# henriChevreux/distillation_trajectories

Hardware: AMD Instinct MI355X
Metric: trajectory-timesteps/sec (B×T U-Net fwd) at 16×16 T=50 (higher is better)
Workload: dtype f32 (fp32-accurate; convolutions: exact 3-plane bf16 operand split on bf16 MFMA with fp32 accumulate, or native fp32 MFMA, chosen per layer)

## Files before the change

distillation_trajectories_amd/csrc/dt_conv.hip:

```cpp
#include "dt_conv_epilogue.h"

namespace dt {

template <int BM, int BN>
__global__ __launch_bounds__(256, 4) void conv_gemm_kernel(const ConvParams p) {
  constexpr ConvForm F = *find_conv_form(KIND_FP32, BM, BN);
  constexpr int WN = F.wn();
  constexpr int MI = F.mi(), NI = F.ni();
  constexpr int A_PER = BM / 64, B_PER = BN / 64;
  constexpr int STAGE = (BM + BN) * 16;
  constexpr int LDS_FLOATS = 2 * STAGE > F.stage_floats() ? 2 * STAGE : F.stage_floats();
  static_assert(F.wm() == 2 && WN == 2 && MI * 64 == BM && NI * 64 == BN && LDS_FLOATS >= F.stage_floats(), "wave layout, epilogue stage");
  __shared__ __attribute__((aligned(16))) float lds[LDS_FLOATS];

  const int tid = threadIdx.x, lane = tid & 63, wave = tid >> 6;
  const int wm = wave / WN, wn = wave % WN;
  const int half = lane >> 5, l31 = lane & 31;
  const int m0 = blockIdx.x * BM, n0 = blockIdx.y * BN;
  const int HW = p.H * p.W;
  const int CC = p.cin_p >> 4;

  int a_off[A_PER], a_off2[A_PER], a_y[A_PER], a_x[A_PER];
  bool a_ok[A_PER];
  int a_lds[A_PER];
#pragma unroll
  for (int j = 0; j < A_PER; ++j) {
    const int q = tid + j * 256, row = q >> 2, pslot = q & 3;
    const int lslot = pslot ^ ((row >> 2) & 3);
    const int m = m0 + row;
    a_ok[j] = m < p.M;
    const int mm = a_ok[j] ? m : 0;
    const int b = mm / HW, rem = mm - b * HW;
    a_y[j] = rem / p.W;
    a_x[j] = rem - a_y[j] * p.W;
    a_off[j] = mm * p.cin_p + lslot * 4;
    a_off2[j] = mm * p.cin2_p + lslot * 4;
    a_lds[j] = q * 4;
  }
  const float *wbase = p.w + (size_t)n0 * 16 + tid * 4;

  f32x16 acc[MI][NI];
#pragma unroll
  for (int mi = 0; mi < MI; ++mi)
#pragma unroll
    for (int ni = 0; ni < NI; ++ni)
#pragma unroll
      for (int r = 0; r < 16; ++r) acc[mi][ni][r] = 0.f;

  int a_row[MI], b_row[NI];
#pragma unroll
  for (int mi = 0; mi < MI; ++mi) a_row[mi] = wm * (MI * 32) + mi * 32 + l31;
#pragma unroll
  for (int ni = 0; ni < NI; ++ni) b_row[ni] = wn * (NI * 32) + ni * 32 + l31;

  const int n_main = (p.tap_hi - p.tap_lo) * CC / p.splits;
  const int n_iter = n_main + (p.in2 ? (p.cin2_p >> 4) : 0);
  int tap = p.tap_lo + (blockIdx.z * n_main) / CC, cc = (blockIdx.z * n_main) % CC;
  for (int it = -1; it < n_iter; ++it) {
    const bool more = it + 1 < n_iter;
    f32x4 ra[A_PER], rb[B_PER];
    if (more && it + 1 >= n_main) {
      const int c2 = it + 1 - n_main;
#pragma unroll
      for (int j = 0; j < A_PER; ++j)
        ra[j] = a_ok[j] ? *reinterpret_cast<const f32x4 *>(p.in2 + a_off2[j] + c2 * 16) : f32x4{0.f, 0.f, 0.f, 0.f};
      const float *wt = p.w2 + (size_t)n0 * 16 + tid * 4 + (size_t)c2 * p.n_p * 16;
#pragma unroll
      for (int j = 0; j < B_PER; ++j) rb[j] = *reinterpret_cast<const f32x4 *>(wt + j * 1024);
    } else if (more) {
      int dy = 0, dx = 0;
      if (p.ksize == 3) { dy = tap / 3 - 1; dx = tap - (tap / 3) * 3 - 1; }
      const int shift = (dy * p.W + dx) * p.cin_p + cc * 16;
#pragma unroll
      for (int j = 0; j < A_PER; ++j) {
        const int yy = a_y[j] + dy, xx = a_x[j] + dx;
        const bool ok = a_ok[j] && yy >= 0 && yy < p.H && xx >= 0 && xx < p.W;
        ra[j] = ok ? *reinterpret_cast<const f32x4 *>(p.in + a_off[j] + shift) : f32x4{0.f, 0.f, 0.f, 0.f};
      }
      const float *wt = wbase + (size_t)(tap * p.ccw + cc) * p.n_p * 16;
#pragma unroll
      for (int j = 0; j < B_PER; ++j) rb[j] = *reinterpret_cast<const f32x4 *>(wt + j * 1024);
      if (++cc == CC) { cc = 0; ++tap; }
    }
    if (it >= 0) {
      if (it == n_main && p.in2) conv_midpoint<MI, NI>(p, acc, n0, wn, l31);
      const float *A = lds + (it & 1) * STAGE, *B = A + BM * 16;
#pragma unroll
      for (int s = 0; s < 2; ++s) {
        f32x4 fa[MI], fb[NI];
#pragma unroll
        for (int mi = 0; mi < MI; ++mi)
          fa[mi] = *reinterpret_cast<const f32x4 *>(A + a_row[mi] * 16 + (((2 * s + half) ^ ((a_row[mi] >> 2) & 3)) << 2));
#pragma unroll
        for (int ni = 0; ni < NI; ++ni)
          fb[ni] = *reinterpret_cast<const f32x4 *>(B + b_row[ni] * 16 + (((2 * s + half) ^ ((b_row[ni] >> 2) & 3)) << 2));
#pragma unroll
        for (int i = 0; i < 4; ++i)
#pragma unroll
          for (int mi = 0; mi < MI; ++mi)
#pragma unroll
            for (int ni = 0; ni < NI; ++ni) {
              acc[mi][ni] = __builtin_amdgcn_mfma_f32_32x32x2f32(fa[mi][i], fb[ni][i], acc[mi][ni], 0, 0, 0);
            }
      }
    }
    if (more) {
      float *A = lds + ((it + 1) & 1) * STAGE, *B = A + BM * 16;
#pragma unroll
      for (int j = 0; j < A_PER; ++j) *reinterpret_cast<f32x4 *>(A + a_lds[j]) = ra[j];
#pragma unroll
      for (int j = 0; j < B_PER; ++j) *reinterpret_cast<f32x4 *>(B + (tid + j * 256) * 4) = rb[j];
    }
    __syncthreads();
  }

  conv_epilogue<BM, BN, 1>(p, acc, lds, m0, n0, wm, wn, half, l31);
}

int launch_splitk_epilogue(const ConvParams &p, hipStream_t s);

#define DT_GEMM_ROW(cls, kind, bm, bn, kc, wk) {{kind, bm, bn, kc, wk, cls}, conv_gemm_kernel<bm, bn>},
static const ConvKernel kGemmKernels[] = {DT_CONV_FORMS_FP32(DT_GEMM_ROW)};

int launch_conv(const ConvParams &p, hipStream_t s) {
  if (!p.in || !p.w || !p.scale || !p.shift || !p.out) return DT_E_NULL;
  if (p.cin_p % 16 || p.cout_p % 16 || p.n_p % kNPad || p.M <= 0) return DT_E_SHAPE;
  if ((long long)p.M * p.cin_p >= (1ll << 31) || (long long)p.M * p.cout_p * (p.n_dup > 1 ? p.n_dup : 1) >= (1ll << 31)) return DT_E_SHAPE;
  if (const int st = conv_admissible(p)) return st;
  {
    const double flops = 2.0 * p.M * (double)p.cout_real * ((double)p.cin_real * p.ksize * p.ksize + (p.in2 ? p.cin2_real : 0));
    ProfileScope prof(find_conv_form(p.kind, p.bm, p.bn)->cls, flops, 4.0 * p.M * ((double)p.cin_real + p.cout_real), s);
    if (p.kind == KIND_FP32) {
      conv_kernel_of(kGemmKernels, p).fn<<<dim3((p.M + p.bm - 1) / p.bm, p.n_p / p.bn, p.splits), 256, 0, s>>>(p);
      DT_LAUNCH_CHECK();
    } else if (const int st = is_strip(p.kind) ? launch_conv_strip(p, s) : launch_conv_bf16x6(p, s)) return st;
  }
  return p.splits > 1 ? launch_splitk_epilogue(p, s) : DT_OK;
}


bool conv_choice_valid(const ConvChoice &c, int slot, int n_p) {
  if (!find_conv_form(c.kind, c.bm, c.bn) || n_p % c.bn) return false;
  if (c.splits < 1 || c.splits > 9 || c.splits == 5 || c.splits == 6 || c.splits == 7) return false;
  return !c.fuse || (slot == 2 && c.splits == 1);
}

static ConvChoice heuristic_choice(int M, int n_p, int taps) {
  ConvChoice c{};
  c.bn = n_p % 128 == 0 ? 128 : 64;
  const long long blocks128 = (long long)((M + 127) / 128) * (n_p / c.bn);
  c.bm = blocks128 >= 512 ? 128 : 64;
  const long long blocks = (long long)((M + c.bm - 1) / c.bm) * (n_p / c.bn);
  c.splits = 1;
  if (taps == 9 && M <= kSplitMaxRows && blocks < 384) c.splits = blocks * 3 >= 384 ? 3 : 9;
  c.fuse = c.splits == 1;
  return c;
}

ConvChoice resolve_conv_choice(const ConvLayer &L, const ConvChoice *req, int precision) {
  ConvChoice c = req ? *req : heuristic_choice(L.M, L.n_p, L.splittable ? L.taps : 1);
  const int cc = L.cin_p >> 4;
  if (!req) {
    c.kind = precision == DT_PREC_FP32 ? KIND_FP32 : KIND_BF16;
    if (c.kind == KIND_BF16 && L.taps == 9 && strip_reaches(L.W)) {
      c.kind = KIND_STRIP;
      c.splits = c.splits == 9 ? (cc % 8 == 0 ? 8 : (cc % 4 == 0 ? 4 : 1)) : (c.splits == 3 ? (cc % 4 == 0 ? 4 : (cc % 2 == 0 ? 2 : 1)) : 1);
    }
  }
  if (c.kind == 2) c.kind = KIND_BF16;
  if (is_strip(c.kind) && (L.taps != 9 || !strip_reaches(L.W))) c.kind = KIND_BF16;
  if (c.kind == KIND_STRIPK && !find_conv_form(c.kind, c.bm, c.bn)) c.kind = KIND_STRIP2;
  if (c.bm == 256 && !find_conv_form(c.kind, c.bm, c.bn)) c.bm = 128;
  if (!L.splittable) c.splits = 1;
  const ConvForm *f = find_conv_form(c.kind, c.bm, c.bn);
  if (is_strip(c.kind) ? !chunks_fit(cc, pack_chunks(L.cin_p), c.splits * (f ? f->kc : 1)) : (L.taps * cc) % c.splits != 0)
    c.splits = 1;
  c.fuse = L.foldable && c.fuse && c.splits == 1;
  return c;
}

int conv_admissible(const ConvParams &p) {
  const int cc = p.cin_p >> 4;
  const ConvForm *f = find_conv_form(p.kind, p.bm, p.bn);
  if (!f || p.n_p % p.bn) return DT_E_ARG;
  if (p.splits < 1 || (p.splits > 1 && !p.slab)) return DT_E_ARG;
  if (p.ccw < cc || (p.in2 && p.ccw2 < (p.cin2_p >> 4))) return DT_E_ARG;
  if (p.in2 && (p.splits != 1 || !p.w2 || !p.bias2 || p.cin2_p % 16)) return DT_E_ARG;
  if (!is_strip(p.kind)) return (p.tap_hi - p.tap_lo) * cc % p.splits ? DT_E_ARG : DT_OK;
  if (p.ksize != 3 || p.tap_lo != 0 || p.tap_hi != 9 || !chunks_fit(cc, p.ccw, p.splits * f->kc)) return DT_E_ARG;
  if (p.in2 && !chunks_fit(p.cin2_p >> 4, p.ccw2, f->kc)) return DT_E_ARG;
  return f->reaches(p.W) ? DT_OK : DT_E_SHAPE;
}

template <int S>
__device__ inline float4 splitk_finish(const ConvParams &p, unsigned m, int n, size_t slab_stride) {
  const size_t o = (size_t)m * p.cout_p + n;
  float4 a;
  if (S > 0) {
    float4 part[S > 0 ? S : 1];
#pragma unroll
    for (int z = 0; z < S; ++z) part[z] = *reinterpret_cast<const float4 *>(p.slab + z * slab_stride + o);
    a = part[0];
#pragma unroll
    for (int z = 1; z < S; ++z) { a.x += part[z].x; a.y += part[z].y; a.z += part[z].z; a.w += part[z].w; }
  } else {
    a = *reinterpret_cast<const float4 *>(p.slab + o);
    for (int z = 1; z < p.splits; ++z) {
      const float4 b = *reinterpret_cast<const float4 *>(p.slab + z * slab_stride + o);
      a.x += b.x; a.y += b.y; a.z += b.z; a.w += b.w;
    }
  }
  const float4 sc = *reinterpret_cast<const float4 *>(p.scale + n), sh = *reinterpret_cast<const float4 *>(p.shift + n);
  float4 v = make_float4(a.x * sc.x + sh.x, a.y * sc.y + sh.y, a.z * sc.z + sh.z, a.w * sc.w + sh.w);
  if (p.relu) { v.x = fmaxf(v.x, 0.f); v.y = fmaxf(v.y, 0.f); v.z = fmaxf(v.z, 0.f); v.w = fmaxf(v.w, 0.f); }
  if (p.tb) {
    const float4 t = *reinterpret_cast<const float4 *>(p.tb + (size_t)(m / (unsigned)p.m_per_tb) * p.tb_stride + n);
    v.x += t.x; v.y += t.y; v.z += t.z; v.w += t.w;
  }
  if (p.add) {
    const float4 t = *reinterpret_cast<const float4 *>(p.add + o);
    v.x += t.x; v.y += t.y; v.z += t.z; v.w += t.w;
  }
  *reinterpret_cast<float4 *>(p.out + o) = v;
  return v;
}

template <int S, bool POOL>
__global__ __launch_bounds__(256) void splitk_epilogue_kernel(const ConvParams p) {
  const unsigned c4 = (unsigned)p.cout_p >> 2;
  const size_t slab_stride = (size_t)p.M * p.cout_p;
  if (!POOL) {
    const unsigned total = (unsigned)p.M * c4;
    const bool pow2 = (c4 & (c4 - 1)) == 0;
    const int sh4 = 31 - __builtin_clz(c4);
    for (unsigned i = blockIdx.x * blockDim.x + threadIdx.x; i < total; i += gridDim.x * blockDim.x) {
      const unsigned m = pow2 ? i >> sh4 : i / c4;
      splitk_finish<S>(p, m, (int)(i - m * c4) * 4, slab_stride);
    }
  } else {
    const unsigned Wo = (unsigned)p.W >> 1, Ho = (unsigned)p.H >> 1, HW = (unsigned)(p.H * p.W);
    const unsigned total = ((unsigned)p.M >> 2) * c4;
    for (unsigned i = blockIdx.x * blockDim.x + threadIdx.x; i < total; i += gridDim.x * blockDim.x) {
      const unsigned wq = i / c4;
      const int n = (int)(i - wq * c4) * 4;
      const unsigned xo = wq % Wo, r = wq / Wo;
      const unsigned yo = r % Ho, b = r / Ho;
      const unsigned m00 = b * HW + 2 * yo * (unsigned)p.W + 2 * xo;
      const float4 a = splitk_finish<S>(p, m00, n, slab_stride), bq = splitk_finish<S>(p, m00 + 1, n, slab_stride);
      const float4 c = splitk_finish<S>(p, m00 + p.W, n, slab_stride), d = splitk_finish<S>(p, m00 + p.W + 1, n, slab_stride);
      float4 mx;
      mx.x = fmaxf(fmaxf(a.x, bq.x), fmaxf(c.x, d.x)); mx.y = fmaxf(fmaxf(a.y, bq.y), fmaxf(c.y, d.y));
      mx.z = fmaxf(fmaxf(a.z, bq.z), fmaxf(c.z, d.z)); mx.w = fmaxf(fmaxf(a.w, bq.w), fmaxf(c.w, d.w));
      *reinterpret_cast<float4 *>(p.pool_out + (size_t)wq * p.cout_p + n) = mx;
    }
  }
}

template <bool POOL>
static int launch_splitk_epilogue_t(const ConvParams &p, hipStream_t s) {
  const size_t total = (size_t)(POOL ? p.M / 4 : p.M) * (p.cout_p / 4);
  const int blocks = (int)((total + 255) / 256 < 4096 ? (total + 255) / 256 : 4096);
  ProfileScope prof(KC_SPLITK_EPILOGUE, 0.0, 4.0 * p.M * p.cout_p * (p.splits + 1.0 + (POOL ? 0.25 : 0.0)), s);
  switch (p.splits) {
    case 2: splitk_epilogue_kernel<2, POOL><<<blocks, 256, 0, s>>>(p); break;
    case 3: splitk_epilogue_kernel<3, POOL><<<blocks, 256, 0, s>>>(p); break;
    case 4: splitk_epilogue_kernel<4, POOL><<<blocks, 256, 0, s>>>(p); break;
    case 8: splitk_epilogue_kernel<8, POOL><<<blocks, 256, 0, s>>>(p); break;
    case 9: splitk_epilogue_kernel<9, POOL><<<blocks, 256, 0, s>>>(p); break;
    default: splitk_epilogue_kernel<0, POOL><<<blocks, 256, 0, s>>>(p); break;
  }
  DT_LAUNCH_CHECK();
  return DT_OK;
}

int launch_splitk_epilogue(const ConvParams &p, hipStream_t s) {
  return p.pool_out ? launch_splitk_epilogue_t<true>(p, s) : launch_splitk_epilogue_t<false>(p, s);
}

__global__ void pack_conv_kernel(const float *__restrict__ w, float *__restrict__ wp, int cout, int cin, int ksize,
                                 int cin_p, int n_p, int split_c, int split_cp, size_t total) {
  for (size_t idx = blockIdx.x * (size_t)blockDim.x + threadIdx.x; idx < total; idx += (size_t)gridDim.x * blockDim.x) {
    const int pos = idx & 15;
    const size_t rowi = idx >> 4;
    const int n = rowi % n_p;
    const int kc = rowi / n_p;
    const int pslot = pos >> 2, e = pos & 3;
    const int lslot = pslot ^ ((n >> 2) & 3);
    const int k = kc * 16 + lslot * 4 + e;
    const int tap = k / cin_p, cp = k - tap * cin_p;
    int c = -1;
    if (cp < split_cp) { if (cp < split_c) c = cp; }
    else { const int cc = split_c + (cp - split_cp); if (cc < cin) c = cc; }
    float v = 0.f;
    if (n < cout && c >= 0) v = w[((size_t)n * cin + c) * (ksize * ksize) + tap];
    wp[idx] = v;
  }
}

int launch_pack_conv(const float *w, float *wp, int cout, int cin, int ksize, int cin_p, int n_p, int split_c,
                     int split_cp, hipStream_t s) {
  const size_t total = (size_t)ksize * ksize * cin_p * n_p;
  const int blocks = (int)((total + 255) / 256 < 4096 ? (total + 255) / 256 : 4096);
  pack_conv_kernel<<<blocks, 256, 0, s>>>(w, wp, cout, cin, ksize, cin_p, n_p, split_c, split_cp, total);
  DT_LAUNCH_CHECK();
  return DT_OK;
}

__global__ void fold_bn_kernel(const float *cb, const float *g, const float *b, const float *mean, const float *var,
                               float *scale, float *shift, int cout, int n_p) {
  const int n = blockIdx.x * blockDim.x + threadIdx.x;
  if (n >= n_p) return;
  float sc = 0.f, sh = 0.f;
  if (n < cout) {
    if (g) {
      sc = g[n] / sqrtf(var[n] + 1e-5f);
      sh = (cb[n] - mean[n]) * sc + b[n];
    } else {
      sc = 1.f;
      sh = cb[n];
    }
  }
  scale[n] = sc;
  shift[n] = sh;
}

int launch_fold_bn(const float *cb, const float *g, const float *b, const float *mean, const float *var, float *scale,
                   float *shift, int cout, int n_p, hipStream_t s) {
  fold_bn_kernel<<<(n_p + 255) / 256, 256, 0, s>>>(cb, g, b, mean, var, scale, shift, cout, n_p);
  DT_LAUNCH_CHECK();
  return DT_OK;
}

__global__ void pack_res3_kernel(const float *w, const float *b, float *w3, int cout, int C, int n_p) {
  const int n = blockIdx.x * blockDim.x + threadIdx.x;
  if (n >= n_p) return;
  float4 v = make_float4(0.f, 0.f, 0.f, 0.f);
  if (n < cout) {
    v.x = w[n * C];
    if (C > 1) v.y = w[n * C + 1];
    if (C > 2) v.z = w[n * C + 2];
    v.w = b[n];
  }
  *reinterpret_cast<float4 *>(w3 + 4 * n) = v;
}

int launch_pack_res3(const float *w, const float *b, float *w3, int cout, int C, int n_p, hipStream_t s) {
  if (C > 3) return DT_E_SHAPE;
  pack_res3_kernel<<<(n_p + 255) / 256, 256, 0, s>>>(w, b, w3, cout, C, n_p);
  DT_LAUNCH_CHECK();
  return DT_OK;
}

}
```

distillation_trajectories_amd/csrc/dt_conv_epilogue.h:

```cpp
#pragma once
#include "dt_internal.h"

namespace dt {

typedef float f32x16 __attribute__((ext_vector_type(16)));
typedef float f32x4 __attribute__((ext_vector_type(4)));

typedef __bf16 bf16x8 __attribute__((ext_vector_type(8)));
typedef __bf16 bf16x2 __attribute__((ext_vector_type(2)));
typedef unsigned u32x4 __attribute__((ext_vector_type(4)));

__device__ inline float bf16_to_f32(__bf16 v) { return (float)v; }

__device__ inline void split8(const f32x4 lo, const f32x4 hi, bf16x8 &p1, bf16x8 &p2, bf16x8 &p3) {
#pragma unroll
  for (int i = 0; i < 8; ++i) {
    const float a = i < 4 ? lo[i] : hi[i - 4];
    const __bf16 a1 = (__bf16)a;
    const float r1 = a - (float)a1;
    const __bf16 a2 = (__bf16)r1;
    const float r2 = r1 - (float)a2;
    p1[i] = a1; p2[i] = a2; p3[i] = (__bf16)r2;
  }
}

__device__ inline void mfma_bf16x6(f32x16 &acc, const bf16x8 (&fa)[3], const bf16x8 (&fb)[3]) {
  f32x16 c = acc;
  c = __builtin_amdgcn_mfma_f32_32x32x16_bf16(fa[2], fb[0], c, 0, 0, 0);
  c = __builtin_amdgcn_mfma_f32_32x32x16_bf16(fa[1], fb[1], c, 0, 0, 0);
  c = __builtin_amdgcn_mfma_f32_32x32x16_bf16(fa[0], fb[2], c, 0, 0, 0);
  c = __builtin_amdgcn_mfma_f32_32x32x16_bf16(fa[1], fb[0], c, 0, 0, 0);
  c = __builtin_amdgcn_mfma_f32_32x32x16_bf16(fa[0], fb[1], c, 0, 0, 0);
  c = __builtin_amdgcn_mfma_f32_32x32x16_bf16(fa[0], fb[0], c, 0, 0, 0);
  acc = c;
}

template <int BM, int BN, int WK, int MI, int NI>
__device__ inline void conv_epilogue(const ConvParams &p, f32x16 (&acc)[MI][NI], float *stage, int m0, int n0, int wm, int wn,
                                     int half, int l31, int wk = 0) {
  constexpr ConvForm F = *find_conv_layout(BM, BN, WK);
  static_assert(MI == F.mi() && NI == F.ni(), "accumulator tiles of the form");
  constexpr int WM = F.wm(), P = F.pitch(), C4 = BN / 4, U = WM * C4 / 8;
  constexpr int COPY = F.copy_floats();
  const int tid = threadIdx.x;
  const int HW = p.H * p.W;
  const bool pow2 = (p.W & (p.W - 1)) == 0 && (HW & (HW - 1)) == 0;
  const int w_sh = 31 - __builtin_clz(p.W), hw_sh = 31 - __builtin_clz(HW);
  auto div_hw = [&](int m) { return pow2 ? m >> hw_sh : m / HW; };
  auto div_w = [&](int r) { return pow2 ? r >> w_sh : r / p.W; };
  const bool slab_mode = p.splits > 1;
  const size_t slab_stride = (size_t)p.M * p.cout_p;
  const int c4 = tid % C4, row0 = tid / C4;
  const int n = n0 + c4 * 4;
  const bool n_ok = n < p.cout_p;
  const int nn = n_ok ? n : 0;
  auto unit = [&](int k) __attribute__((always_inline)) {
    const float *src = stage + (row0 + k * (256 / C4)) * P + c4 * 4;
    f32x4 v = *reinterpret_cast<const f32x4 *>(src);
#pragma unroll
    for (int c = 1; c < WK; ++c) v += *reinterpret_cast<const f32x4 *>(src + c * COPY);
    return v;
  };
  auto unit_row = [&](int mi, int k) { const int row = row0 + k * (256 / C4); return m0 + (row >> 5) * (MI * 32) + mi * 32 + (row & 31); };
  auto to_stage = [&](int mi) __attribute__((always_inline)) {
    __syncthreads();
#pragma unroll
    for (int ni = 0; ni < NI; ++ni)
#pragma unroll
      for (int r = 0; r < 16; ++r) {
        const int L = 4 * half + (r & 3) + 8 * (r >> 2);
        stage[wk * COPY + (wm * 32 + L) * P + wn * (NI * 32) + ni * 32 + l31] = acc[mi][ni][r];
      }
    __syncthreads();
  };

  if (slab_mode) {
    float *slab = p.slab + (size_t)blockIdx.z * slab_stride;
#pragma unroll
    for (int mi = 0; mi < MI; ++mi) {
      to_stage(mi);
#pragma unroll
      for (int k = 0; k < U; ++k) {
        const int m = unit_row(mi, k);
        if (n_ok && m < p.M)
          *reinterpret_cast<f32x4 *>(slab + (size_t)m * p.cout_p + n) = unit(k);
      }
    }
    return;
  }

  auto pool_pass = [&](int mi, float *pool_out, const float *src, int n_src, int src_pitch, size_t out_pitch) __attribute__((always_inline)) {
    __syncthreads();
    const int Wo = p.W >> 1;
    for (int q0 = tid; q0 < n_src * WM * 8 * C4; q0 += 256) {
      const int pass = q0 / (WM * 8 * C4), q = q0 - pass * (WM * 8 * C4);
      const int pp = q / C4, qc = q % C4, j = pp & 7;
      const int yy = pow2 ? j >> (w_sh - 1) : j / Wo, xx = j - yy * Wo;
      const int L0 = 2 * yy * p.W + 2 * xx;
      const int m = m0 + (pp >> 3) * (MI * 32) + mi * 32 + L0;
      const int qn = n0 + qc * 4;
      if (m >= p.M || qn >= p.cout_p || (pass && m < p.dup_skip)) continue;
      const float *s0 = src + pass * src_pitch + ((pp >> 3) * 32 + L0) * P + qc * 4;
      const f32x4 a = *reinterpret_cast<const f32x4 *>(s0), b = *reinterpret_cast<const f32x4 *>(s0 + P);
      const f32x4 c = *reinterpret_cast<const f32x4 *>(s0 + p.W * P), d = *reinterpret_cast<const f32x4 *>(s0 + (p.W + 1) * P);
      f32x4 mx;
#pragma unroll
      for (int e = 0; e < 4; ++e) mx[e] = fmaxf(fmaxf(a[e], b[e]), fmaxf(c[e], d[e]));
      const int bimg = div_hw(m), rem = m - bimg * HW;
      const int y = div_w(rem), x = rem - y * p.W;
      *reinterpret_cast<f32x4 *>(pool_out + pass * out_pitch + (((size_t)bimg * (p.H >> 1) + (y >> 1)) * Wo + (x >> 1)) * p.cout_p + qn) = mx;
    }
  };
  f32x4 w3r[4];
#pragma unroll
  for (int e = 0; e < 4; ++e) w3r[e] = p.x3 ? *reinterpret_cast<const f32x4 *>(p.w3 + 4 * (nn + e)) : f32x4{0.f, 0.f, 0.f, 0.f};
  auto x3_skip = [&](int m, int) __attribute__((always_inline)) {
    f32x4 r;
    const int img = div_hw(m), pix = m - img * HW;
    const float *xr = p.x3 + (size_t)(img < p.x3_imgs ? img : img % p.x3_imgs) * p.x3_c * p.x3_hw + pix;
    const float x0 = xr[0], x1 = p.x3_c > 1 ? xr[p.x3_hw] : 0.f, x2 = p.x3_c > 2 ? xr[2 * p.x3_hw] : 0.f;
#pragma unroll
    for (int e = 0; e < 4; ++e) {
      const f32x4 w3 = w3r[e];
      float rs = w3[3];
      rs = fmaf(x0, w3[0], rs);
      if (p.x3_c > 1) rs = fmaf(x1, w3[1], rs);
      if (p.x3_c > 2) rs = fmaf(x2, w3[2], rs);
      r[e] = rs;
    }
    return r;
  };

#pragma unroll
  for (int mi = 0; mi < MI; ++mi) {
    f32x4 v[U];
    int mrow[U];
    bool ok[U];
    to_stage(mi);
#pragma unroll
    for (int k = 0; k < U; ++k) {
      mrow[k] = unit_row(mi, k);
      ok[k] = n_ok && mrow[k] < p.M;
    }
#pragma unroll
    for (int k = 0; k < U; ++k) v[k] = unit(k);
    if (p.n_dup) {
      const f32x4 sc = *reinterpret_cast<const f32x4 *>(p.scale + nn), sh = *reinterpret_cast<const f32x4 *>(p.shift + nn);
      f32x4 rs[U];
      int cls[U], mc[U];
#pragma unroll
      for (int k = 0; k < U; ++k) {
        mc[k] = ok[k] ? mrow[k] : m0;
        const int pix = mc[k] - div_hw(mc[k]) * HW, y = div_w(pix), x = pix - y * p.W;
        cls[k] = 3 * (y == 0 ? 0 : (y == p.H - 1 ? 2 : 1)) + (x == 0 ? 0 : (x == p.W - 1 ? 2 : 1));
      }
#pragma unroll
      for (int k = 0; k < U; ++k) rs[k] = p.x3 ? x3_skip(mc[k], nn) : f32x4{0.f, 0.f, 0.f, 0.f};
      if (p.n_dup == 2 && p.dup_stage2 && p.pool_out) {
        float *stage2 = stage + WK * COPY;
        f32x4 b0[U], b1[U];
#pragma unroll
        for (int k = 0; k < U; ++k) {
          const unsigned r0 = (unsigned)mc[k] / (unsigned)p.m_per_tb;
          const unsigned r1 = (unsigned)(p.dup_rows + (mc[k] >= p.dup_skip ? mc[k] - p.dup_skip : mc[k])) / (unsigned)p.m_per_tb;
          b0[k] = *reinterpret_cast<const f32x4 *>(p.tbc + (size_t)r0 * p.tb_stride + cls[k] * p.cout_p + nn);
          b1[k] = *reinterpret_cast<const f32x4 *>(p.tbc + (size_t)r1 * p.tb_stride + cls[k] * p.cout_p + nn);
        }
#pragma unroll
        for (int k = 0; k < U; ++k) {
          f32x4 o0 = (v[k] + b0[k]) * sc + sh, o1 = (v[k] + b1[k]) * sc + sh;
          if (p.relu) {
#pragma unroll
            for (int e = 0; e < 4; ++e) { o0[e] = fmaxf(o0[e], 0.f); o1[e] = fmaxf(o1[e], 0.f); }
          }
          o0 += rs[k]; o1 += rs[k];
          if (ok[k] && !p.skip_out) {
            *reinterpret_cast<f32x4 *>(p.out + (size_t)mrow[k] * p.cout_p + n) = o0;
            if (mrow[k] >= p.dup_skip) *reinterpret_cast<f32x4 *>(p.out + ((size_t)p.dup_rows + mrow[k] - p.dup_skip) * p.cout_p + n) = o1;
          }
          *reinterpret_cast<f32x4 *>(stage + (row0 + k * (256 / C4)) * P + c4 * 4) = o0;
          *reinterpret_cast<f32x4 *>(stage2 + (row0 + k * (256 / C4)) * P + c4 * 4) = o1;
        }
        pool_pass(mi, p.pool_out, stage, 2, WK * COPY, (size_t)((p.dup_rows - p.dup_skip) >> 2) * p.cout_p);
        continue;
      }
      for (int pass = 0; pass < p.n_dup; ++pass) {
        if (pass && m0 < p.dup_skip) break;
        f32x4 o[U];
        const int shift = pass ? pass * p.dup_rows - p.dup_skip : 0;
#pragma unroll
        for (int k = 0; k < U; ++k) {
          o[k] = f32x4{0.f, 0.f, 0.f, 0.f};
          if (ok[k]) {
            const size_t mg = (size_t)shift + mrow[k];
            const unsigned tr = (unsigned)(shift + mrow[k]) / (unsigned)p.m_per_tb;
            const f32x4 b = *reinterpret_cast<const f32x4 *>(p.tbc + (size_t)tr * p.tb_stride + cls[k] * p.cout_p + n);
            o[k] = (v[k] + b) * sc + sh;
            if (p.relu) {
#pragma unroll
              for (int e = 0; e < 4; ++e) o[k][e] = fmaxf(o[k][e], 0.f);
            }
            o[k] += rs[k];
            if (!p.skip_out) *reinterpret_cast<f32x4 *>(p.out + mg * p.cout_p + n) = o[k];
          }
        }
        if (p.pool_out) {
          if (pass) __syncthreads();
#pragma unroll
          for (int k = 0; k < U; ++k) *reinterpret_cast<f32x4 *>(stage + (row0 + k * (256 / C4)) * P + c4 * 4) = o[k];
          pool_pass(mi, p.pool_out + (size_t)(shift >> 2) * p.cout_p, stage, 1, 0, 0);
        }
      }
      continue;
    }
    if (p.in2) {
      const f32x4 b2 = *reinterpret_cast<const f32x4 *>(p.bias2 + nn);
#pragma unroll
      for (int k = 0; k < U; ++k) v[k] += b2;
    } else {
      const f32x4 sc = *reinterpret_cast<const f32x4 *>(p.scale + nn), sh = *reinterpret_cast<const f32x4 *>(p.shift + nn);
#pragma unroll
      for (int k = 0; k < U; ++k) {
        v[k] = v[k] * sc + sh;
        if (p.relu) {
#pragma unroll
          for (int e = 0; e < 4; ++e) v[k][e] = fmaxf(v[k][e], 0.f);
        }
      }
    }
    if (p.tb) {
      f32x4 t[U];
#pragma unroll
      for (int k = 0; k < U; ++k) {
        t[k] = f32x4{0.f, 0.f, 0.f, 0.f};
        if (ok[k]) t[k] = *reinterpret_cast<const f32x4 *>(p.tb + (size_t)(mrow[k] / p.m_per_tb) * p.tb_stride + n);
      }
#pragma unroll
      for (int k = 0; k < U; ++k) v[k] += t[k];
    }
    if (p.add) {
      f32x4 a[U];
#pragma unroll
      for (int k = 0; k < U; ++k) {
        a[k] = f32x4{0.f, 0.f, 0.f, 0.f};
        if (ok[k]) a[k] = *reinterpret_cast<const f32x4 *>(p.add + (size_t)mrow[k] * p.cout_p + n);
      }
#pragma unroll
      for (int k = 0; k < U; ++k) v[k] += a[k];
    }
    if (p.x3) {
#pragma unroll
      for (int k = 0; k < U; ++k)
        if (ok[k]) v[k] += x3_skip(mrow[k], nn);
    }
    if (p.head_out) {
      f32x4 hw[3];
#pragma unroll
      for (int c = 0; c < 3; ++c) {
        hw[c] = f32x4{0.f, 0.f, 0.f, 0.f};
        if (c < p.head_c && n_ok) {
#pragma unroll
          for (int e = 0; e < 4; ++e)
            if (n + e < p.head_cin) hw[c][e] = p.head_w[c * p.head_cin + n + e];
        }
      }
#pragma unroll
      for (int k = 0; k < U; ++k) {
        float part[3];
#pragma unroll
        for (int c = 0; c < 3; ++c) {
          part[c] = 0.f;
#pragma unroll
          for (int e = 0; e < 4; ++e) part[c] = fmaf(hw[c][e], v[k][e], part[c]);
#pragma unroll
          for (int off = C4 / 2; off > 0; off >>= 1) part[c] += __shfl_xor(part[c], off, 64);
        }
        if (c4 == 0 && mrow[k] < p.M) {
          f32x4 o = {part[0] + p.head_b[0], 0.f, 0.f, 0.f};
          if (p.head_c > 1) o[1] = part[1] + p.head_b[1];
          if (p.head_c > 2) o[2] = part[2] + p.head_b[2];
          *reinterpret_cast<f32x4 *>(p.head_out + (size_t)mrow[k] * 4) = o;
        }
      }
      continue;
    }
#pragma unroll
    for (int k = 0; k < U; ++k)
      if (ok[k]) *reinterpret_cast<f32x4 *>(p.out + (size_t)mrow[k] * p.cout_p + n) = v[k];
    if (p.pool_out) {
#pragma unroll
      for (int k = 0; k < U; ++k) *reinterpret_cast<f32x4 *>(stage + (row0 + k * (256 / C4)) * P + c4 * 4) = v[k];
      pool_pass(mi, p.pool_out, stage, 1, 0, 0);
    }
  }
}

template <int MI, int NI>
__device__ inline void conv_midpoint(const ConvParams &p, f32x16 (&acc)[MI][NI], int n0, int wn, int l31) {
#pragma unroll
  for (int ni = 0; ni < NI; ++ni) {
    const int n = n0 + wn * (NI * 32) + ni * 32 + l31;
    const float sc = p.scale[n], sh = p.shift[n];
#pragma unroll
    for (int mi = 0; mi < MI; ++mi)
#pragma unroll
      for (int r = 0; r < 16; ++r) {
        const float v = acc[mi][ni][r] * sc + sh;
        acc[mi][ni][r] = p.relu ? fmaxf(v, 0.f) : v;
      }
  }
}

}
```

distillation_trajectories_amd/csrc/dt_internal.h:

```cpp
#pragma once
#include <hip/hip_runtime.h>
#include <stddef.h>
#include <stdint.h>

#include "../../include/dt_hip.h"
#include "dt_conv_forms.h"

#define DT_HIP_TRY(expr)                         \
  do {                                           \
    hipError_t _e = (expr);                      \
    if (_e != hipSuccess) return (int)_e;        \
  } while (0)
#define DT_LAUNCH_CHECK()                        \
  do {                                           \
    hipError_t _e = hipGetLastError();           \
    if (_e != hipSuccess) return (int)_e;        \
  } while (0)

namespace dt {

enum KernelClass {
  KC_SPLITK_EPILOGUE = KC_CONV_COUNT, KC_FIRST_CONV, KC_POOL, KC_UPCAT, KC_HEAD, KC_HEAD_UP, KC_TIME_BIAS, KC_UPDATE, KC_METRICS,
  KC_WASSERSTEIN, KC_RESAMPLE, KC_FUSED, KC_PAIR_METRICS,
  KC_COUNT
};
struct ProfileScope {
  ProfileScope(int cls, double flops, double bytes, hipStream_t s);
  ~ProfileScope();
  int slot;
  hipStream_t stream;
  void *end_event;
};

__device__ inline void bilinear_src(int dst, int in, int out, int &i0, int &i1, float &l0, float &l1) {
#pragma clang fp contract(off)
  const float scale = out > 1 ? (float)(in - 1) / (float)(out - 1) : 0.f;
  const float src = scale * (float)dst;
  i0 = (int)src;
  i1 = i0 + (i0 < in - 1 ? 1 : 0);
  l1 = src - (float)i0;
  l0 = 1.f - l1;
}
__device__ inline float bilinear_blend(float v00, float v01, float v10, float v11, float wy0, float wy1, float wx0, float wx1) {
  const float top = fmaf(wx1, v01, wx0 * v00), bot = fmaf(wx1, v11, wx0 * v10);
  return fmaf(wy1, bot, wy0 * top);
}

constexpr int kChanPad = 16;
constexpr int kNPad = 64;
constexpr int kBlocks = 8;
constexpr int kChunkPad = 4;

inline int round_up(int v, int m) { return (v + m - 1) / m * m; }
inline bool chunks_fit(int cc, int ccw, int div) { return div >= 1 && round_up(cc, div) <= ccw; }
inline int pack_chunks(int cin_p) { return round_up(cin_p, 16 * kChunkPad) >> 4; }

struct ConvParams {
  const float *in;
  const float *w;
  const float *scale;
  const float *shift;
  const float *tb;
  const float *add;
  float *out;
  int M, H, W;
  int cin_p, cout_p, n_p;
  int cin_real, cout_real;
  int ksize;
  int tap_lo, tap_hi;
  int relu;
  int tb_stride;
  int m_per_tb;
  int splits;
  float *slab;
  int bm, bn;
  int kind;
  const float *x3;
  const float *w3;
  int x3_hw, x3_imgs, x3_c;
  const float *in2;
  const float *w2;
  const float *bias2;
  int cin2_p, cin2_real;
  float *pool_out;
  const float *in_b, *in2_b;
  int cc_a, b_stride;
  const float *head_w, *head_b;
  float *head_out;
  int head_c, head_cin;
  const float *tbc;
  int n_dup, dup_rows;
  int dup_skip;
  int skip_out;
  int dup_stage2;
  int ccw, ccw2;
};

int launch_conv(const ConvParams &p, hipStream_t s);
int launch_conv_bf16x6(const ConvParams &p, hipStream_t s);
int launch_conv_strip(const ConvParams &p, hipStream_t s);
struct ConvKernel { ConvForm form; void (*fn)(ConvParams); };
template <size_t N>
inline const ConvKernel &conv_kernel_of(const ConvKernel (&table)[N], const ConvParams &p) {
  for (const ConvKernel &k : table)
    if (k.form.kind == p.kind && k.form.bm == p.bm && k.form.bn == p.bn) return k;
  return table[0];
}
int launch_pack_conv_bf16x3(const float *w_oihw, void *wp, int cout, int cin, int ksize, int cin_p, int cin_w, int n_p,
                            int split_c, int split_cp, hipStream_t s);
constexpr int kSplitMaxRows = 32768;

struct ConvChoice { int bm, bn, splits, kind, fuse; };
struct ConvLayer {
  int M, W;
  int n_p, cin_p;
  int taps;
  bool splittable;
  bool foldable;
};
inline bool strip_reaches(int W) { return find_conv_form(KIND_STRIP, 64, 64)->reaches(W); }
bool conv_choice_valid(const ConvChoice &c, int slot, int n_p);
ConvChoice resolve_conv_choice(const ConvLayer &L, const ConvChoice *req, int precision);
int conv_admissible(const ConvParams &p);

int launch_pack_conv(const float *w_oihw, float *wp, int cout, int cin, int ksize, int cin_p, int n_p,
                     int split_c, int split_cp, hipStream_t s);
int launch_fold_bn(const float *conv_b, const float *g, const float *b, const float *mean, const float *var,
                   float *scale, float *shift, int cout, int n_p, hipStream_t s);
int launch_pack_linear_rows(const float *w, const float *b, float *wp, float *bp, int out, int in, int out_p,
                            hipStream_t s);

int launch_first_conv(const float *x, const float *wf, const float *scale, const float *shift, const float *tb, int tb_stride,
                      int tb_div, float *out, int B, int n_pass, int C, int H, int W, int cout, int cout_p, hipStream_t s);
int launch_pack_first_conv(const float *w_oihw, float *wf, int cout, int C, int cout_p, hipStream_t s);
int launch_pack_tap_major(const float *w_oihw, float *w2t, int cout, int cin, int cp, hipStream_t s);
int launch_maxpool(const float *in, float *out, int Bt, int H, int W, int cp, hipStream_t s);
int launch_upcat(const float *lo, const float *skip, float *out, int Bt, int h, int w, int c1p, int c2p,
                 hipStream_t s);
int launch_head(const float *lo, const float *w, const float *bias, float *lowres, int Bt, int h, int w_, int cp, int C, int c_real,
                hipStream_t s);
int launch_head_upsample(const float *lowres, float *eps, int Bt, int h, int w_, int C, hipStream_t s);
int launch_pack_res3(const float *w, const float *b, float *w3, int cout, int C, int n_p, hipStream_t s);
int launch_cfg_update_lowres(int rule, const float *x, const float *lowres_u, const float *lowres_c, const float *z,
                             const int32_t *z_row, long long z_shift, const float coef[4], int has_noise, const float *w,
                             float w_scalar, float *out, int B, int C, int H, int W, int b_single, hipStream_t s);

struct TembWeights {
  const float *freqs;
  const float *w1, *b1;
  const float *wc0, *bc0;
  const float *wc2, *bc2;
  const float *wt, *bt;
  int D, half, tb_stride;
  int tb_cols;
  const float *w2t;
  int c0p;
};
int launch_time_bias(const TembWeights &tw, const int32_t *t, const float *cond, const uint8_t *present, int rows,
                     float *out, hipStream_t s);

}
```

distillation_trajectories_amd/csrc/dt_layers.hip:

```cpp
#include "dt_conv_epilogue.h"

namespace dt {

template <int C, int PX>
__global__ __launch_bounds__(256) void first_conv_kernel(const float *__restrict__ x, const float *__restrict__ wf,
                                                         const float *__restrict__ scale, const float *__restrict__ shift,
                                                         const float *__restrict__ tb, int tb_stride, int tb_div,
                                                         float *__restrict__ out, int B, int n_pass, int H, int W, int cp,
                                                         int parts) {
  extern __shared__ float img[];
  const int tid = threadIdx.x, b = blockIdx.x / parts, part = blockIdx.x - b * parts;
  const int Wp = W + 2, plane = (H + 2) * Wp, HW = H * W;
  const int QN = cp >> 2, PPI = 256 / QN;
  const int q = tid % QN, pl = tid / QN;
  f32x4 w[9 * C];
#pragma unroll
  for (int k = 0; k < 9 * C; ++k) w[k] = *reinterpret_cast<const f32x4 *>(wf + (size_t)k * cp + q * 4);
  const f32x4 sc = *reinterpret_cast<const f32x4 *>(scale + q * 4), sh = *reinterpret_cast<const f32x4 *>(shift + q * 4);
  for (int i = tid; i < C * plane; i += 256) {
    const int c = i / plane, r = i - c * plane;
    const int y = r / Wp - 1, xx = r - (y + 1) * Wp - 1;
    img[i] = (y >= 0 && y < H && xx >= 0 && xx < W) ? x[((size_t)(b * C + c) * H + y) * W + xx] : 0.f;
  }
  __syncthreads();
  if (pl >= PPI) return;
  const int GW = W / PX, G = H * GW;
  const int per = (G + parts - 1) / parts;
  const int hi = (part + 1) * per < G ? (part + 1) * per : G;
  for (int g = part * per + pl; g < hi; g += PPI) {
    const int y = g / GW, x0 = (g - y * GW) * PX;
    f32x4 acc[PX];
#pragma unroll
    for (int px = 0; px < PX; ++px) acc[px] = f32x4{0.f, 0.f, 0.f, 0.f};
#pragma unroll
    for (int c = 0; c < C; ++c)
#pragma unroll
      for (int dy = 0; dy < 3; ++dy) {
        float v[PX + 2];
#pragma unroll
        for (int j = 0; j < PX + 2; ++j) v[j] = img[c * plane + (y + dy) * Wp + x0 + j];
#pragma unroll
        for (int dx = 0; dx < 3; ++dx)
#pragma unroll
          for (int px = 0; px < PX; ++px)
#pragma unroll
            for (int e = 0; e < 4; ++e) acc[px][e] = fmaf(v[px + dx], w[c * 9 + dy * 3 + dx][e], acc[px][e]);
      }
#pragma unroll
    for (int px = 0; px < PX; ++px)
#pragma unroll
      for (int e = 0; e < 4; ++e) acc[px][e] = fmaxf(acc[px][e] * sc[e] + sh[e], 0.f);
    const int pix = y * W + x0;
    for (int pass = 0; pass < n_pass; ++pass) {
      const int bt = pass * B + b;
      const f32x4 t = tb ? *reinterpret_cast<const f32x4 *>(tb + (size_t)(bt / tb_div) * tb_stride + q * 4) : f32x4{0.f, 0.f, 0.f, 0.f};
#pragma unroll
      for (int px = 0; px < PX; ++px)
        *reinterpret_cast<f32x4 *>(out + ((size_t)bt * HW + pix + px) * cp + q * 4) = acc[px] + t;
    }
  }
}

template <int PX>
static void first_conv_dispatch(int C, int grid, size_t lds, hipStream_t s, const float *x, const float *wf, const float *scale,
                                const float *shift, const float *tb, int tb_stride, int tb_div, float *out, int B, int n_pass,
                                int H, int W, int cout_p, int parts) {
  if (C == 1) first_conv_kernel<1, PX><<<grid, 256, lds, s>>>(x, wf, scale, shift, tb, tb_stride, tb_div, out, B, n_pass, H, W, cout_p, parts);
  else if (C == 2) first_conv_kernel<2, PX><<<grid, 256, lds, s>>>(x, wf, scale, shift, tb, tb_stride, tb_div, out, B, n_pass, H, W, cout_p, parts);
  else first_conv_kernel<3, PX><<<grid, 256, lds, s>>>(x, wf, scale, shift, tb, tb_stride, tb_div, out, B, n_pass, H, W, cout_p, parts);
}

int launch_first_conv(const float *x, const float *wf, const float *scale, const float *shift, const float *tb, int tb_stride,
                      int tb_div, float *out, int B, int n_pass, int C, int H, int W, int cout, int cout_p, hipStream_t s) {
  if (C < 1 || C > 3 || cout_p % 4 || cout_p > 1024) return DT_E_SHAPE;
  const size_t lds = (size_t)C * (H + 2) * (W + 2) * sizeof(float);
  if (lds > 64 * 1024) return DT_E_SHAPE;
  const int parts = B >= 1024 ? 1 : (B >= 256 ? 4 : 8);
  ProfileScope prof(KC_FIRST_CONV, 2.0 * n_pass * B * H * W * (double)cout * 9 * C, 4.0 * B * H * W * (C + (double)n_pass * cout_p), s);
  if (W % 4 == 0) first_conv_dispatch<4>(C, B * parts, lds, s, x, wf, scale, shift, tb, tb_stride, tb_div, out, B, n_pass, H, W, cout_p, parts);
  else first_conv_dispatch<1>(C, B * parts, lds, s, x, wf, scale, shift, tb, tb_stride, tb_div, out, B, n_pass, H, W, cout_p, parts);
  DT_LAUNCH_CHECK();
  return DT_OK;
}

__global__ void pack_first_conv_kernel(const float *__restrict__ w, float *__restrict__ wf, int cout, int C, int cp) {
  const int i = blockIdx.x * blockDim.x + threadIdx.x;
  if (i >= 9 * C * cp) return;
  const int k = i / cp, n = i - k * cp;
  wf[i] = n < cout ? w[(size_t)n * 9 * C + k] : 0.f;
}

int launch_pack_first_conv(const float *w_oihw, float *wf, int cout, int C, int cout_p, hipStream_t s) {
  pack_first_conv_kernel<<<(9 * C * cout_p + 255) / 256, 256, 0, s>>>(w_oihw, wf, cout, C, cout_p);
  DT_LAUNCH_CHECK();
  return DT_OK;
}

__global__ void maxpool_kernel(const float4 *__restrict__ in, float4 *__restrict__ out, int Bt, int H, int W,
                               int c4) {
  const int Ho = H >> 1, Wo = W >> 1;
  const size_t total = (size_t)Bt * Ho * Wo * c4;
  for (size_t i = blockIdx.x * (size_t)blockDim.x + threadIdx.x; i < total; i += (size_t)gridDim.x * blockDim.x) {
    const int c = i % c4;
    size_t r = i / c4;
    const int xo = r % Wo; r /= Wo;
    const int yo = r % Ho;
    const int b = r / Ho;
    const float4 *p = in + (((size_t)b * H + 2 * yo) * W + 2 * xo) * c4 + c;
    const float4 a = p[0], bq = p[c4], cq = p[(size_t)W * c4], d = p[(size_t)W * c4 + c4];
    float4 o;
    o.x = fmaxf(fmaxf(a.x, bq.x), fmaxf(cq.x, d.x));
    o.y = fmaxf(fmaxf(a.y, bq.y), fmaxf(cq.y, d.y));
    o.z = fmaxf(fmaxf(a.z, bq.z), fmaxf(cq.z, d.z));
    o.w = fmaxf(fmaxf(a.w, bq.w), fmaxf(cq.w, d.w));
    out[i] = o;
  }
}

int launch_maxpool(const float *in, float *out, int Bt, int H, int W, int cp, hipStream_t s) {
  const size_t total = (size_t)Bt * (H / 2) * (W / 2) * (cp / 4);
  const int blocks = (int)((total + 255) / 256 < 2048 ? (total + 255) / 256 : 2048);
  ProfileScope prof(KC_POOL, 0.0, 4.0 * Bt * H * W * cp * 1.25, s);
  maxpool_kernel<<<blocks, 256, 0, s>>>(reinterpret_cast<const float4 *>(in), reinterpret_cast<float4 *>(out), Bt,
                                         H, W, cp / 4);
  DT_LAUNCH_CHECK();
  return DT_OK;
}

__global__ __launch_bounds__(256) void upcat_kernel(const float4 *__restrict__ lo, const float4 *__restrict__ skip,
                                                    float4 *__restrict__ out, int Bt, int h, int w, int c1q, int c2q) {
  const unsigned H = 2 * h, W = 2 * w, cq = c1q + c2q;
  const unsigned cw = skip ? cq : (unsigned)c1q;
  const unsigned total = (unsigned)Bt * H * W * cw;
  for (unsigned i = blockIdx.x * blockDim.x + threadIdx.x; i < total; i += gridDim.x * blockDim.x) {
    const unsigned pixel = i / cw, c = i - pixel * cw;
    const unsigned row = pixel / W, x = pixel - row * W;
    const unsigned b = row / H, y = row - b * H;
    float4 o;
    if (c >= (unsigned)c1q) {
      o = skip[(size_t)pixel * c2q + (c - c1q)];
    } else {
      int y0, y1, x0, x1;
      float wy0, wy1, wx0, wx1;
      bilinear_src((int)y, h, (int)H, y0, y1, wy0, wy1);
      bilinear_src((int)x, w, (int)W, x0, x1, wx0, wx1);
      const float4 *base = lo + (size_t)b * h * w * c1q + c;
      const float4 v00 = base[(y0 * w + x0) * c1q], v01 = base[(y0 * w + x1) * c1q];
      const float4 v10 = base[(y1 * w + x0) * c1q], v11 = base[(y1 * w + x1) * c1q];
      o.x = wy0 * (wx0 * v00.x + wx1 * v01.x) + wy1 * (wx0 * v10.x + wx1 * v11.x);
      o.y = wy0 * (wx0 * v00.y + wx1 * v01.y) + wy1 * (wx0 * v10.y + wx1 * v11.y);
      o.z = wy0 * (wx0 * v00.z + wx1 * v01.z) + wy1 * (wx0 * v10.z + wx1 * v11.z);
      o.w = wy0 * (wx0 * v00.w + wx1 * v01.w) + wy1 * (wx0 * v10.w + wx1 * v11.w);
    }
    out[(size_t)pixel * cq + c] = o;
  }
}

int launch_upcat(const float *lo, const float *skip, float *out, int Bt, int h, int w, int c1p, int c2p,
                 hipStream_t s) {
  const size_t total = (size_t)Bt * 4 * h * w * ((c1p + (skip ? c2p : 0)) / 4);
  if (total >= (1ull << 32)) return DT_E_SHAPE;
  const int blocks = (int)((total + 255) / 256 < 8192 ? (total + 255) / 256 : 8192);
  ProfileScope prof(KC_UPCAT, 0.0, 4.0 * Bt * h * w * (c1p + 4.0 * c1p + (skip ? 8.0 * c2p : 0.0)), s);
  upcat_kernel<<<blocks, 256, 0, s>>>(reinterpret_cast<const float4 *>(lo), reinterpret_cast<const float4 *>(skip),
                                       reinterpret_cast<float4 *>(out), Bt, h, w, c1p / 4, c2p / 4);
  DT_LAUNCH_CHECK();
  return DT_OK;
}

__global__ __launch_bounds__(256) void head_kernel(const float *__restrict__ lo, const float *__restrict__ wf,
                                                   const float *__restrict__ bias, float *__restrict__ lowres,
                                                   size_t n_pix, int cp, int C, int c_real) {
  const int sub = threadIdx.x & 7;
  const size_t g0 = (blockIdx.x * (size_t)blockDim.x + threadIdx.x) >> 3;
  const size_t n_groups = ((size_t)gridDim.x * blockDim.x) >> 3;
  const int c4 = cp >> 2;
  for (size_t base = g0 - (g0 & 7); base < n_pix; base += n_groups) {
    const size_t pix = base + (g0 & 7);
    float part[4] = {0.f, 0.f, 0.f, 0.f};
    if (pix < n_pix) {
      const float4 *p4 = reinterpret_cast<const float4 *>(lo + pix * cp);
      for (int q = sub; q < c4; q += 8) {
        const float4 v = p4[q];
        const float vv[4] = {v.x, v.y, v.z, v.w};
#pragma unroll
        for (int e = 0; e < 4; ++e) {
          const int k = q * 4 + e;
          if (k < c_real) {
#pragma unroll
            for (int c = 0; c < 4; ++c)
              if (c < C) part[c] = fmaf(wf[c * c_real + k], vv[e], part[c]);
          }
        }
      }
    }
#pragma unroll
    for (int c = 0; c < 4; ++c)
#pragma unroll
      for (int off = 4; off > 0; off >>= 1) part[c] += __shfl_xor(part[c], off, 64);
    if (sub == 0 && pix < n_pix) {
      float4 o = make_float4(part[0] + bias[0], 0.f, 0.f, 0.f);
      if (C > 1) o.y = part[1] + bias[1];
      if (C > 2) o.z = part[2] + bias[2];
      *reinterpret_cast<float4 *>(lowres + pix * 4) = o;
    }
  }
}

__global__ void head_upsample_kernel(const float *__restrict__ lowres, float *__restrict__ eps, int Bt, int h, int w,
                                     int C) {
  const int H = 2 * h, W = 2 * w;
  const size_t total = (size_t)Bt * C * H * W;
  for (size_t i = blockIdx.x * (size_t)blockDim.x + threadIdx.x; i < total; i += (size_t)gridDim.x * blockDim.x) {
    const int x = i % W;
    size_t r = i / W;
    const int y = r % H; r /= H;
    const int c = r % C;
    const size_t b = r / C;
    int y0, y1, x0, x1;
    float wy0, wy1, wx0, wx1;
    bilinear_src(y, h, H, y0, y1, wy0, wy1);
    bilinear_src(x, w, W, x0, x1, wx0, wx1);
    const float *base = lowres + b * h * w * 4 + c;
    const float v00 = base[((size_t)y0 * w + x0) * 4], v01 = base[((size_t)y0 * w + x1) * 4];
    const float v10 = base[((size_t)y1 * w + x0) * 4], v11 = base[((size_t)y1 * w + x1) * 4];
    eps[i] = bilinear_blend(v00, v01, v10, v11, wy0, wy1, wx0, wx1);
  }
}

__global__ __launch_bounds__(256) void resize_bilinear_kernel(const float *__restrict__ in, float *__restrict__ out, int planes,
                                                              int h, int w, int H, int W) {
  const int Wq = (W + 3) >> 2;
  const size_t total = (size_t)planes * H * Wq;
  for (size_t i = blockIdx.x * (size_t)blockDim.x + threadIdx.x; i < total; i += (size_t)gridDim.x * blockDim.x) {
    const int xq = i % Wq;
    size_t r = i / Wq;
    const int y = r % H;
    const size_t pl = r / H;
    int y0, y1;
    float wy0, wy1;
    bilinear_src(y, h, H, y0, y1, wy0, wy1);
    const float *base = in + pl * (size_t)h * w;
    float v[4];
#pragma unroll
    for (int j = 0; j < 4; ++j) {
      const int x = xq * 4 + j;
      v[j] = 0.f;
      if (x < W) {
        int x0, x1;
        float wx0, wx1;
        bilinear_src(x, w, W, x0, x1, wx0, wx1);
        v[j] = bilinear_blend(base[(size_t)y0 * w + x0], base[(size_t)y0 * w + x1], base[(size_t)y1 * w + x0], base[(size_t)y1 * w + x1],
                              wy0, wy1, wx0, wx1);
      }
    }
    float *o = out + (pl * H + y) * (size_t)W + xq * 4;
    if (W % 4 == 0) *reinterpret_cast<float4 *>(o) = make_float4(v[0], v[1], v[2], v[3]);
    else
      for (int j = 0; j < 4 && xq * 4 + j < W; ++j) o[j] = v[j];
  }
}

extern "C" int dt_resize_bilinear(const float *in, float *out, int planes, int h, int w, int H, int W, void *stream) {
  hipStream_t s = (hipStream_t)stream;
  if (!in || !out) return DT_E_NULL;
  if (planes < 1 || h < 1 || w < 1 || H < 1 || W < 1) return DT_E_SHAPE;
  const size_t total = (size_t)planes * H * ((W + 3) / 4);
  const int blocks = (int)((total + 255) / 256 < 4096 ? (total + 255) / 256 : 4096);
  ProfileScope prof(KC_POOL, 0.0, 4.0 * planes * ((double)h * w + (double)H * W), s);
  resize_bilinear_kernel<<<blocks, 256, 0, s>>>(in, out, planes, h, w, H, W);
  DT_LAUNCH_CHECK();
  return DT_OK;
}

int launch_head(const float *lo, const float *wf, const float *bias, float *lowres, int Bt, int h, int w, int cp, int C, int c_real,
                hipStream_t s) {
  if (C > 3) return DT_E_SHAPE;
  const size_t n_pix = (size_t)Bt * h * w;
  const size_t blocks = (n_pix + 31) / 32;
  ProfileScope prof(KC_HEAD, 2.0 * n_pix * C * c_real, 4.0 * n_pix * (c_real + 4.0), s);
  head_kernel<<<(int)(blocks < 8192 ? blocks : 8192), 256, 0, s>>>(lo, wf, bias, lowres, n_pix, cp, C, c_real);
  DT_LAUNCH_CHECK();
  return DT_OK;
}

int launch_head_upsample(const float *lowres, float *eps, int Bt, int h, int w, int C, hipStream_t s) {
  const size_t n_pix = (size_t)Bt * h * w;
  const size_t total = n_pix * 4 * C;
  const int blocks = (int)((total + 255) / 256 < 2048 ? (total + 255) / 256 : 2048);
  ProfileScope prof(KC_HEAD_UP, 0.0, 4.0 * n_pix * (4.0 + 4.0 * C), s);
  head_upsample_kernel<<<blocks, 256, 0, s>>>(lowres, eps, Bt, h, w, C);
  DT_LAUNCH_CHECK();
  return DT_OK;
}

template <int G>
__device__ inline void wave_dots(const float *__restrict__ w, int ld, const float *vec, int n, int lane, int count, float (&res)[G]) {
  float s[G];
#pragma unroll
  for (int j = 0; j < G; ++j) s[j] = 0.f;
  for (int k = lane; k < n; k += 64) {
    const float v = vec[k];
#pragma unroll
    for (int j = 0; j < G; ++j)
      if (j < count) s[j] = fmaf(w[(size_t)j * ld + k], v, s[j]);
  }
#pragma unroll
  for (int j = 0; j < G; ++j) {
    for (int off = 32; off > 0; off >>= 1) s[j] += __shfl_down(s[j], off, 64);
    res[j] = __shfl(s[j], 0, 64);
  }
}

__global__ __launch_bounds__(1024) void time_bias_kernel(const TembWeights tw, const int32_t *__restrict__ t,
                                                         const float *__restrict__ cond,
                                                         const uint8_t *__restrict__ present, float *__restrict__ out,
                                                         int slices) {
  extern __shared__ float sm[];
  constexpr int G = 4;
  const int D = tw.D, row = blockIdx.x / slices, slice = blockIdx.x - row * slices;
  float *emb = sm, *hid = sm + D, *temb = sm + 2 * D;
  const int tid = threadIdx.x, lane = tid & 63, wave = tid >> 6, n_waves = blockDim.x >> 6;
  const float tv = (float)t[row];
  for (int k = tid; k < D; k += blockDim.x) {
    float v = 0.f;
    if (k < tw.half) v = sinf(tv * tw.freqs[k]);
    else if (k < 2 * tw.half) v = cosf(tv * tw.freqs[k - tw.half]);
    emb[k] = v;
  }
  const bool has_cond = cond != nullptr && (present == nullptr || present[row] != 0);
  const float cv = has_cond ? cond[row] : 0.f;
  for (int k = tid; k < D; k += blockDim.x) hid[k] = fmaxf(fmaf(tw.wc0[k], cv, tw.bc0[k]), 0.f);
  __syncthreads();
  for (int o = wave * G; o < D; o += n_waves * G) {
    const int cnt = D - o < G ? D - o : G;
    float a[G], b[G];
    wave_dots<G>(tw.w1 + (size_t)o * D, D, emb, D, lane, cnt, a);
    if (has_cond) wave_dots<G>(tw.wc2 + (size_t)o * D, D, hid, D, lane, cnt, b);
    if (lane == 0)
      for (int j = 0; j < cnt; ++j) {
        float v = fmaxf(a[j] + tw.b1[o + j], 0.f);
        if (has_cond) v += b[j] + tw.bc2[o + j];
        temb[o + j] = v;
      }
  }
  __syncthreads();
  float *orow = out + (size_t)row * tw.tb_stride;
  const int per = (tw.tb_cols + slices - 1) / slices;
  const int lo = slice * per, hi = lo + per < tw.tb_cols ? lo + per : tw.tb_cols;
  for (int o = lo + wave * G; o < hi; o += n_waves * G) {
    const int cnt = hi - o < G ? hi - o : G;
    float a[G];
    wave_dots<G>(tw.wt + (size_t)o * D, D, temb, D, lane, cnt, a);
    if (lane == 0)
      for (int j = 0; j < cnt; ++j) orow[o + j] = fmaxf(a[j] + tw.bt[o + j], 0.f);
  }
}

__global__ __launch_bounds__(1024) void tap_bias_kernel(const TembWeights tw, float *__restrict__ out) {
  extern __shared__ float bsm[];
  const int c0p = tw.c0p;
  float *tsum = bsm + c0p;
  float *orow = out + (size_t)blockIdx.x * tw.tb_stride;
  for (int i = threadIdx.x; i < c0p; i += blockDim.x) bsm[i] = orow[i];
  __syncthreads();
  for (int i = threadIdx.x; i < 9 * c0p; i += blockDim.x) {
    const int tap = i / c0p, n = i - tap * c0p;
    const float *w = tw.w2t + (size_t)tap * c0p * c0p + n;
    float a = 0.f;
    for (int ci = 0; ci < c0p; ++ci) a = fmaf(w[(size_t)ci * c0p], bsm[ci], a);
    tsum[i] = a;
  }
  __syncthreads();
  for (int i = threadIdx.x; i < 9 * c0p; i += blockDim.x) {
    const int cls = i / c0p, n = i - cls * c0p;
    const int cy = cls / 3, cx = cls - 3 * cy;
    float a = 0.f;
#pragma unroll
    for (int tap = 0; tap < 9; ++tap) {
      const int dy = tap / 3 - 1, dx = tap % 3 - 1;
      const bool in = !(cy == 0 && dy < 0) && !(cy == 2 && dy > 0) && !(cx == 0 && dx < 0) && !(cx == 2 && dx > 0);
      if (in) a += tsum[tap * c0p + n];
    }
    orow[tw.tb_cols + i] = a;
  }
}

int launch_time_bias(const TembWeights &tw, const int32_t *t, const float *cond, const uint8_t *present, int rows,
                     float *out, hipStream_t s) {
  if (rows <= 0) return DT_OK;
  const int slices = rows >= 512 ? 1 : (rows >= 64 ? 4 : 8);
  ProfileScope prof(KC_TIME_BIAS, 2.0 * rows * tw.D * (2.0 * tw.D + tw.tb_cols) + (tw.w2t ? 18.0 * rows * tw.c0p * tw.c0p : 0.0),
                    4.0 * rows * tw.tb_stride, s);
  time_bias_kernel<<<rows * slices, 1024, 3 * tw.D * sizeof(float), s>>>(tw, t, cond, present, out, slices);
  DT_LAUNCH_CHECK();
  if (tw.w2t) {
    tap_bias_kernel<<<rows, 1024, 10 * tw.c0p * sizeof(float), s>>>(tw, out);
    DT_LAUNCH_CHECK();
  }
  return DT_OK;
}

__global__ void pack_tap_major_kernel(const float *__restrict__ w, float *__restrict__ w2t, int cout, int cin, int cp) {
  const int i = blockIdx.x * blockDim.x + threadIdx.x;
  if (i >= 9 * cp * cp) return;
  const int n = i % cp, ci = (i / cp) % cp, tap = i / (cp * cp);
  w2t[i] = (n < cout && ci < cin) ? w[((size_t)n * cin + ci) * 9 + tap] : 0.f;
}

int launch_pack_tap_major(const float *w_oihw, float *w2t, int cout, int cin, int cp, hipStream_t s) {
  pack_tap_major_kernel<<<(9 * cp * cp + 255) / 256, 256, 0, s>>>(w_oihw, w2t, cout, cin, cp);
  DT_LAUNCH_CHECK();
  return DT_OK;
}

__global__ void pack_linear_rows_kernel(const float *w, const float *b, float *wp, float *bp, int out, int in, int out_p) {
  const size_t total = (size_t)out_p * in;
  for (size_t i = blockIdx.x * (size_t)blockDim.x + threadIdx.x; i < total; i += (size_t)gridDim.x * blockDim.x) {
    const int o = i / in;
    wp[i] = o < out ? w[i] : 0.f;
    if (i % in == 0) bp[o] = o < out ? b[o] : 0.f;
  }
}

int launch_pack_linear_rows(const float *w, const float *b, float *wp, float *bp, int out, int in, int out_p,
                            hipStream_t s) {
  const size_t total = (size_t)out_p * in;
  pack_linear_rows_kernel<<<(int)((total + 255) / 256), 256, 0, s>>>(w, b, wp, bp, out, in, out_p);
  DT_LAUNCH_CHECK();
  return DT_OK;
}

}
```

distillation_trajectories_amd/csrc/dt_unet.hip:

```cpp
#include <algorithm>
#include <atomic>
#include <cstdio>
#include <cstdlib>
#include <cstring>
#include <mutex>
#include <new>
#include <vector>

#include "dt_fused.h"
#include "dt_internal.h"

using namespace dt;

namespace {
struct ProfRecord { hipEvent_t a, b; int cls; double flops, bytes; };
struct Profiler {
  std::mutex mu;
  std::atomic<bool> on{false};
  std::vector<ProfRecord> rec;
  std::vector<hipEvent_t> pool;
  size_t used = 0;
  hipEvent_t get() {
    if (used == pool.size()) {
      hipEvent_t e;
      if (hipEventCreate(&e) != hipSuccess) return nullptr;
      pool.push_back(e);
    }
    return pool[used++];
  }
} g_prof;
const char *kClassName[KC_COUNT - KC_CONV_COUNT] = {
    "splitk_epilogue_kernel", "first_conv_kernel", "maxpool_kernel", "upcat_kernel", "head_kernel", "head_upsample_kernel",
    "time_bias_kernel", "cfg_update_kernel", "traj_metrics_kernel", "wasserstein_kernel", "resampled_distance_kernel",
    "unet_fused_kernel", "pair_metrics_kernel"};
const char *class_name(int cls) {
  switch (cls) {
#define DT_GEMM(c, kind, bm, bn, kc, wk) case c: return "conv_gemm_kernel<" #bm "," #bn ">";
#define DT_BF16(c, kind, bm, bn, kc, wk) case c: return "conv_gemm_bf16x6_kernel<" #bm "," #bn ">";
#define DT_STRIP(c, kind, bm, bn, kc, wk) case c: return "conv_strip_bf16x6_kernel<" #bm "," #bn ">";
#define DT_STRIPK(c, kind, bm, bn, kc, wk) case c: return "conv_strip_bf16x6_kernel<" #bm "," #bn ",K" #kc ">";
    DT_CONV_FORMS_FP32(DT_GEMM) DT_CONV_FORMS_BF16(DT_BF16) DT_CONV_FORMS_STRIP(DT_STRIP) DT_CONV_FORMS_STRIPK(DT_STRIPK)
    default: return kClassName[cls - KC_CONV_COUNT];
  }
}
}

namespace dt {
ProfileScope::ProfileScope(int cls, double flops, double bytes, hipStream_t s) : slot(-1), stream(s), end_event(nullptr) {
  if (!g_prof.on.load(std::memory_order_relaxed)) return;
  hipEvent_t a;
  {
    std::lock_guard<std::mutex> lock(g_prof.mu);
    if (!g_prof.on.load(std::memory_order_relaxed)) return;
    a = g_prof.get();
    hipEvent_t b = g_prof.get();
    if (!a || !b) return;
    g_prof.rec.push_back(ProfRecord{a, b, cls, flops, bytes});
    slot = (int)g_prof.rec.size() - 1;
    end_event = b;
  }
  (void)hipEventRecord(a, s);
}
ProfileScope::~ProfileScope() {
  if (slot < 0) return;
  (void)hipEventRecord((hipEvent_t)end_event, stream);
}
}

struct BlockW {
  int cin, cout;
  int cin_p, cout_p, n_p;
  int split_c, split_cp;
  int cin_w, cout_w;
  bool has_res;
  float *w1, *w2, *wr;
  float *w1b, *w2b, *wrb;
  float *s1, *h1, *s2, *h2, *sr, *hr;
  float *w3;
  int tb_off;
};

struct FwdShape {
  int Bt, H, W, imgs, single;
  static FwdShape rows_only(int Bt, int H, int W) { return FwdShape{Bt, H, W, Bt, 0}; }
  bool operator==(const FwdShape &o) const { return Bt == o.Bt && H == o.H && W == o.W && imgs == o.imgs && single == o.single; }
  int validate() const {
    if (Bt < 1 || imgs < 1 || H < 16 || W < 16 || H % 16 || W % 16) return DT_E_SHAPE;
    if (single < 0 || single >= imgs || (single ? Bt != 2 * imgs - single : Bt % imgs != 0)) return DT_E_ARG;
    return DT_OK;
  }
};

struct TunedShape {
  FwdShape shape;
  ConvChoice c[kBlocks][3];
};

struct LoopGraph {
  std::vector<unsigned char> key;
  hipGraphExec_t exec;
  hipGraph_t graph;
};

struct dt_unet {
  std::vector<TunedShape> tuned;
  mutable std::vector<LoopGraph> graphs;
  mutable std::mutex graph_mu;
  int precision;
  bool head_fusion = true;
  bool share_enc1 = true;
  int tb_cols = 0;
  dt_unet_desc desc;
  BlockW blk[kBlocks];
  int cp[4];
  int tb_stride;
  float *slab;
  size_t slab_floats;
  TembWeights tw;
  const float *final_w, *final_b;
  bool fused_ok = false, fused_on = false;
  int fused_G = 2;
  float *fused_slab = nullptr;
  FusedOp *fused_ops_dev = nullptr;
  int fused_n_ops = 0;
  FusedLds fused_lds{};
  int fused_par = 0, fused_n_par = 0;
};

namespace {

struct Bump {
  size_t off = 0;
  size_t take(size_t n) { size_t o = off; off += (n + 63) / 64 * 64; return o; }
};

bool use_fused(const dt_unet *u, int H, int W);
void fused_common(const dt_unet *u, FusedArgs &a, int B, int n_pass, int B_single, const float *tb, int tb_div);

struct Plan {
  size_t h[kBlocks], r[kBlocks], o[kBlocks];
  size_t pool[4], cat[3];
  size_t slab, lowres;
  size_t total;
  int H[kBlocks], W[kBlocks];
};

const int kDiv[kBlocks] = {1, 2, 4, 8, 16, 8, 4, 2};

Plan make_plan(const dt_unet *u, const FwdShape &sh) {
  const int Bt = sh.Bt, H = sh.H, W = sh.W;
  Plan p{};
  Bump b;
  size_t slab = 0;
  for (int j = 0; j < kBlocks; ++j) {
    const int h = H / kDiv[j], w = W / kDiv[j];
    p.H[j] = h; p.W[j] = w;
    const size_t px = (size_t)Bt * h * w;
    if (j >= 1 && j <= 4) p.pool[j - 1] = b.take(px * u->blk[j].cin_p);
    if (j >= 5) p.cat[j - 5] = b.take(px * u->blk[j].cin_p);
    p.h[j] = b.take(px * u->blk[j].cout_p);
    p.r[j] = (u->blk[j].has_res && j > 0) ? b.take(px * u->blk[j].cout_p) : 0;
    p.o[j] = b.take(px * u->blk[j].cout_p);
    if (j > 0 && px <= (size_t)kSplitMaxRows) {
      const size_t need = (size_t)9 * px * u->blk[j].cout_p;
      if (need > slab) slab = need;
    }
  }
  p.slab = b.take(slab);
  p.lowres = b.take((size_t)Bt * (H / 2) * (W / 2) * 4);
  p.total = b.off;
  return p;
}

void drop_graphs(dt_unet *u) {
  std::lock_guard<std::mutex> lock(u->graph_mu);
  for (LoopGraph &g : u->graphs) { (void)hipGraphExecDestroy(g.exec); (void)hipGraphDestroy(g.graph); }
  u->graphs.clear();
}

const TunedShape *find_tuned(const dt_unet *u, const FwdShape &sh) {
  for (const TunedShape &t : u->tuned)
    if (t.shape == sh) return &t;
  return nullptr;
}

struct ResolvedForward {
  FwdShape shape;
  bool shared_enc1;
  ConvChoice c[kBlocks][3];
  bool pool_fused[kBlocks];
  bool concat_in_place[kBlocks];
  bool head_fused;
};

bool has_launch(const dt_unet *u, int j, int slot) { return slot == 2 || (j > 0 && (slot == 1 || u->blk[j].has_res)); }

ConvLayer conv_layer(const dt_unet *u, const ResolvedForward &f, int j, int slot) {
  const BlockW &k = u->blk[j];
  const int h = f.shape.H / kDiv[j], w = f.shape.W / kDiv[j];
  const int M = (j == 0 && f.shared_enc1 ? f.shape.imgs : f.shape.Bt) * h * w;
  const int taps = slot == 0 || (h == 1 && w == 1) ? 1 : 9;
  return ConvLayer{M, w, k.n_p, slot == 2 ? k.cout_p : k.cin_p, taps, j > 0 && M <= kSplitMaxRows, slot == 2 && j > 0 && k.has_res};
}

ResolvedForward resolve_forward(const dt_unet *u, const FwdShape &sh, const TunedShape *tuned) {
  ResolvedForward f{};
  f.shape = sh;
  f.shared_enc1 = u->share_enc1 && (sh.Bt + sh.single) % sh.imgs == 0;
  for (int j = 0; j < kBlocks; ++j)
    for (int slot = 0; slot < 3; ++slot)
      if (has_launch(u, j, slot)) f.c[j][slot] = resolve_conv_choice(conv_layer(u, f, j, slot), tuned ? &tuned->c[j][slot] : nullptr, u->precision);
  for (int j = 0; j < kBlocks; ++j) {
    const ConvChoice &c2 = f.c[j][2];
    const int h = sh.H / kDiv[j], w = sh.W / kDiv[j];
    f.pool_fused[j] = j <= 3 && h % 2 == 0 && w % 2 == 0 && (c2.splits > 1 || (w <= 16 && (w & (w - 1)) == 0));
    f.concat_in_place[j] = j >= 5 && u->blk[j].has_res && is_strip(f.c[j][1].kind) && is_strip(c2.kind) && c2.fuse;
  }
  const ConvChoice &last = f.c[kBlocks - 1][2];
  f.head_fused = u->head_fusion && last.splits == 1 && u->blk[kBlocks - 1].n_p == last.bn && u->desc.channels <= 3;
  return f;
}

ConvParams bind_conv(const dt_unet *u, const ResolvedForward &f, int j, int slot, const ConvChoice &c, const float *in, float *ws,
                     const Plan &pl, const float *tb, int tb_div) {
  const BlockW &k = u->blk[j];
  const ConvLayer L = conv_layer(u, f, j, slot);
  const int h = pl.H[j], w = pl.W[j];
  ConvParams p{};
  p.M = L.M; p.H = h; p.W = w;
  p.cin_p = L.cin_p; p.cout_p = k.cout_p; p.n_p = k.n_p;
  p.cin_real = slot == 2 ? k.cout : k.cin; p.cout_real = k.cout;
  p.tb_stride = u->tb_stride; p.m_per_tb = h * w * tb_div;
  p.slab = ws + pl.slab;
  p.in = slot == 2 ? ws + pl.h[j] : in;
  p.ksize = slot == 0 ? 1 : 3;
  p.tap_lo = slot > 0 && L.taps == 1 ? 4 : 0; p.tap_hi = p.tap_lo + L.taps;
  p.relu = slot > 0;
  if (slot == 0) {
    p.scale = k.sr; p.shift = k.hr; p.out = ws + pl.r[j];
  } else if (slot == 1) {
    p.scale = k.s1; p.shift = k.h1; p.tb = tb + k.tb_off; p.out = ws + pl.h[j];
  } else {
    p.scale = k.s2; p.shift = k.h2; p.out = ws + pl.o[j];
    if (f.pool_fused[j]) p.pool_out = ws + pl.pool[j];
    if (j == 0) {
      p.x3 = in; p.w3 = k.w3; p.x3_hw = h * w; p.x3_imgs = f.shape.imgs; p.x3_c = u->desc.channels;
      if (f.shared_enc1) {
        p.n_dup = (f.shape.Bt + f.shape.single) / f.shape.imgs; p.dup_rows = p.M; p.dup_skip = f.shape.single * h * w; p.tbc = tb + u->tb_cols;
        p.skip_out = u->head_fusion && p.pool_out ? 1 : 0;
      }
    } else {
      p.add = k.has_res ? ws + pl.r[j] : in;
    }
    if (j == kBlocks - 1 && f.head_fused) {
      p.head_w = u->final_w; p.head_b = u->final_b; p.head_out = ws + pl.lowres;
      p.head_c = u->desc.channels; p.head_cin = u->desc.dims[0];
    }
  }
  const bool fp32 = c.kind == KIND_FP32;
  p.bm = c.bm; p.bn = c.bn; p.splits = c.splits; p.kind = c.kind;
  p.w = slot == 0 ? (fp32 ? k.wr : k.wrb) : (slot == 1 ? (fp32 ? k.w1 : k.w1b) : (fp32 ? k.w2 : k.w2b));
  p.ccw = fp32 ? p.cin_p >> 4 : pack_chunks(p.cin_p);
  if (c.fuse) {
    p.add = nullptr;
    p.in2 = in; p.w2 = fp32 ? k.wr : k.wrb; p.bias2 = k.hr; p.cin2_p = k.cin_p; p.cin2_real = k.cin;
    p.ccw2 = fp32 ? k.cin_p >> 4 : k.cin_w >> 4;
  }
  return p;
}

int run_block(const dt_unet *u, const ResolvedForward &f, int j, const float *in, float *ws, const Plan &pl, const float *tb,
              int tb_div, hipStream_t s) {
  if (j == 0) {
    const BlockW &k = u->blk[0];
    if (!f.shared_enc1 && f.shape.single) return DT_E_ARG;
    const int st = launch_first_conv(in, k.w1, k.s1, k.h1, f.shared_enc1 ? nullptr : tb + k.tb_off, u->tb_stride, tb_div, ws + pl.h[0],
                                     f.shape.imgs, f.shared_enc1 ? 1 : f.shape.Bt / f.shape.imgs, u->desc.channels, pl.H[0], pl.W[0], k.cout, k.cout_p, s);
    if (st) return st;
  }
  for (int slot = 0; slot < 3; ++slot) {
    if (!has_launch(u, j, slot) || (slot == 0 && f.c[j][2].fuse)) continue;
    ConvParams p = bind_conv(u, f, j, slot, f.c[j][slot], in, ws, pl, tb, tb_div);
    if (f.concat_in_place[j]) {
      const int skip = 8 - j;
      p.cc_a = u->blk[j].split_cp >> 4;
      p.b_stride = u->blk[skip].cout_p;
      if (slot == 1) p.in_b = ws + pl.o[skip];
      if (slot == 2) p.in2_b = ws + pl.o[skip];
    }
    const int st = launch_conv(p, s);
    if (st) return st;
  }
  return DT_OK;
}

int forward_impl(const dt_unet *u, const float *x, int B, int n_pass, int H, int W, const float *tb, int tb_div,
                 float *eps, float *ws, size_t ws_bytes, hipStream_t s, int B_single = 0) {
  if (!u || !x || !tb || !ws) return DT_E_NULL;
  if (n_pass < 1 || tb_div < 1) return DT_E_SHAPE;
  const int Bt = B * n_pass - B_single * (n_pass - 1);
  const FwdShape sh{Bt, H, W, B, B_single};
  if (const int bad = sh.validate()) return bad;
  const Plan pl = make_plan(u, sh);
  if (pl.total * sizeof(float) > ws_bytes) return DT_E_WORKSPACE;
  if (use_fused(u, H, W) && eps) {
    if (Bt % tb_div) return DT_E_ARG;
    FusedArgs a{};
    fused_common(u, a, B, n_pass, B_single, tb, tb_div);
    a.mode = FUSED_FORWARD; a.x = x; a.eps = eps;
    return launch_unet_fused(a, s);
  }
  const ResolvedForward f = resolve_forward(u, sh, find_tuned(u, sh));
  int st = DT_OK;
  const float *cur = x;
  for (int j = 0; j < kBlocks; ++j) {
    if (j >= 1 && j <= 4) {
      if (!f.pool_fused[j - 1])
      st = launch_maxpool(ws + pl.o[j - 1], ws + pl.pool[j - 1], Bt,
                          pl.H[j - 1], pl.W[j - 1], u->blk[j - 1].cout_p, s);
      if (st) return st;
      cur = ws + pl.pool[j - 1];
    } else if (j >= 5) {
      const int skip = 8 - j;
      st = launch_upcat(ws + pl.o[j - 1], f.concat_in_place[j] ? nullptr : ws + pl.o[skip], ws + pl.cat[j - 5],
                        Bt, pl.H[j - 1], pl.W[j - 1], u->blk[j - 1].cout_p, u->blk[skip].cout_p, s);
      if (st) return st;
      cur = ws + pl.cat[j - 5];
    }
    st = run_block(u, f, j, cur, ws, pl, tb, tb_div, s);
    if (st) return st;
  }
  if (!f.head_fused) {
    st = launch_head(ws + pl.o[7], u->final_w, u->final_b, ws + pl.lowres, Bt, pl.H[7], pl.W[7], u->blk[7].cout_p,
                     u->desc.channels, u->desc.dims[0], s);
    if (st) return st;
  }
  if (!eps) return DT_OK;
  return launch_head_upsample(ws + pl.lowres, eps, Bt, pl.H[7], pl.W[7], u->desc.channels, s);
}


int build_fused(dt_unet *u, const float *const *bt, hipStream_t s) {
  const int C = u->desc.channels, c0p = u->cp[0], c1p = u->cp[1];
  if (u->cp[2] != c1p || u->cp[3] != c1p || u->desc.dims[2] != u->desc.dims[1] || u->desc.dims[3] != u->desc.dims[1]) return DT_OK;
  if (!fused_eligible(C, c0p, c1p)) return DT_OK;
  const int G = u->fused_G;
  if (fused_lds_bytes(G, c0p, c1p) > 160 * 1024) return DT_OK;
  Bump bump;
  const int tb_cols = 2 * c0p + 6 * c1p;
  const size_t o_par = bump.take((size_t)5 * tb_cols + 4 * c0p);
  size_t o1[kBlocks] = {}, o2[kBlocks] = {}, orr[kBlocks] = {};
  for (int j = 0; j < kBlocks; ++j) {
    const BlockW &k = u->blk[j];
    if (j > 0) o1[j] = bump.take((size_t)9 * k.cin_p * k.cout_p);
    o2[j] = bump.take((size_t)9 * k.cout_p * k.cout_p);
    if (k.has_res && j > 0) orr[j] = bump.take((size_t)k.cin_p * k.cout_p);
  }
  const size_t o_wf = bump.take((size_t)2 * (c0p / 16) * 256);
  const size_t o_ops = bump.take((sizeof(FusedOp) * kFusedMaxOps + 3) / 4);
  if (bump.off >= (1u << 30)) return DT_OK;
  hipError_t e = hipMalloc((void **)&u->fused_slab, bump.off * sizeof(float));
  if (e != hipSuccess) return (int)e;
  float *F = u->fused_slab;
  FusedModel m{};
  m.c0p = c0p; m.c1p = c1p; m.wf = (int)o_wf; m.w3 = 5 * tb_cols;
  int st = DT_OK;
  auto d2d = [&](size_t off, const float *src, size_t n) {
    if (st == DT_OK) {
      const hipError_t ee = hipMemcpyAsync(F + off, src, n * sizeof(float), hipMemcpyDeviceToDevice, s);
      if (ee != hipSuccess) st = (int)ee;
    }
  };
  st = launch_pack_fused_first(bt[DT_BT_CONV1_W], F + o_wf, u->blk[0].cout, C, c0p / 16, s);
  d2d(o_par + 5 * tb_cols, u->blk[0].w3, (size_t)4 * c0p);
  int pj = 0;
  for (int j = 0; j < kBlocks && st == DT_OK; ++j) {
    const BlockW &k = u->blk[j];
    const float *const *t = bt + j * DT_BT_COUNT;
    FusedBlockW &f = m.blk[j];
    const int cp = k.cout_p;
    d2d(o_par + pj, k.s1, cp); d2d(o_par + pj + cp, k.h1, cp); d2d(o_par + pj + 2 * cp, k.s2, cp); d2d(o_par + pj + 3 * cp, k.h2, cp);
    if (k.has_res && j > 0) d2d(o_par + pj + 4 * cp, k.hr, cp);
    f.tb_off = k.tb_off;
    f.c1 = FusedConvW{(int)o1[j], pj, pj + cp};
    f.c2 = FusedConvW{(int)o2[j], pj + 2 * cp, pj + 3 * cp};
    f.cr = FusedConvW{(int)orr[j], 0, pj + 4 * cp};
    pj += 5 * cp;
    if (j > 0) st = launch_pack_fused_conv(t[DT_BT_CONV1_W], F + o1[j], k.cout, k.cin, 9, k.cin_p / 16, k.cout_p / 16, k.split_c, k.split_cp, s);
    if (!st) st = launch_pack_fused_conv(t[DT_BT_CONV2_W], F + o2[j], k.cout, k.cout, 9, k.cout_p / 16, k.cout_p / 16, k.cout, k.cout_p, s);
    if (!st && k.has_res && j > 0)
      st = launch_pack_fused_conv(t[DT_BT_RES_W], F + orr[j], k.cout, k.cin, 1, k.cin_p / 16, k.cout_p / 16, k.split_c, k.split_cp, s);
  }
  if (st == DT_OK && hipMemsetAsync(F + o_par + 4 * c0p, 0, sizeof(float) * c0p, s) != hipSuccess) st = (int)hipGetLastError();
  u->fused_par = (int)o_par; u->fused_n_par = 5 * tb_cols + 4 * c0p;
  if (st != DT_OK) return st;
  FusedOp ops[kFusedMaxOps];
  u->fused_n_ops = fused_ops(m, G, ops);
  u->fused_ops_dev = reinterpret_cast<FusedOp *>(F + o_ops);
  e = hipMemcpy(u->fused_ops_dev, ops, sizeof(FusedOp) * u->fused_n_ops, hipMemcpyHostToDevice);
  if (e != hipSuccess) return (int)e;
  u->fused_lds = fused_lds(G, c0p, c1p);
  u->fused_ok = true;
  u->fused_on = getenv("DT_NO_FUSED") == nullptr;
  return DT_OK;
}

bool use_fused(const dt_unet *u, int H, int W) { return u->fused_ok && u->fused_on && u->head_fusion && H == 16 && W == 16; }

void fused_common(const dt_unet *u, FusedArgs &a, int B, int n_pass, int B_single, const float *tb, int tb_div) {
  a.ops = u->fused_ops_dev; a.n_ops = u->fused_n_ops; a.fbase = u->fused_slab; a.par = u->fused_par; a.n_par = u->fused_n_par;
  a.head_w = u->final_w; a.head_b = u->final_b;
  a.tb = tb; a.tb_stride = u->tb_stride; a.tb_div = tb_div;
  a.lds = u->fused_lds; a.G = u->fused_G;
  a.C = u->desc.channels; a.c0 = u->desc.dims[0]; a.c0p = u->cp[0];
  a.B = B; a.n_pass = n_pass; a.B_single = B_single;
  a.tb_rows = (B * n_pass - B_single * (n_pass - 1)) / tb_div;
  a.flops_per_row = fused_flops_per_row(a.C, u->desc.dims[0], u->desc.dims[1]);
}

struct ConvTimer {
  hipEvent_t e0 = nullptr, e1 = nullptr;
  ~ConvTimer() {
    if (e0) (void)hipEventDestroy(e0);
    if (e1) (void)hipEventDestroy(e1);
  }
  int create() {
    DT_HIP_TRY(hipEventCreate(&e0));
    DT_HIP_TRY(hipEventCreate(&e1));
    return DT_OK;
  }
  int time(const ConvParams &q, int reps, hipStream_t s, float *ms) {
    *ms = 0.f;
    int st = launch_conv(q, s);
    if (st != DT_OK) return st;
    (void)hipEventRecord(e0, s);
    for (int rep = 0; rep < reps && st == DT_OK; ++rep) st = launch_conv(q, s);
    (void)hipEventRecord(e1, s);
    if (hipEventSynchronize(e1) != hipSuccess) st = (int)hipGetLastError();
    if (st != DT_OK) return st;
    (void)hipEventElapsedTime(ms, e0, e1);
    *ms /= reps;
    return DT_OK;
  }
};

bool slot_exists(int block, int slot) { return block >= 0 && block < kBlocks && slot >= 0 && slot <= 2; }
}

extern "C" {

int dt_abi_version(void) { return DT_ABI_VERSION; }

const char *dt_status_string(int st) {
  switch (st) {
    case DT_OK: return "ok";
    case DT_E_NULL: return "required pointer is NULL";
    case DT_E_SHAPE: return "unsupported or inconsistent shape";
    case DT_E_ARG: return "bad enum or count";
    case DT_E_WORKSPACE: return "workspace too small";
    default: return st > 0 ? hipGetErrorString((hipError_t)st) : "unknown dt status";
  }
}

int dt_unet_create(const dt_unet_desc *desc, const float *const *bt, const float *const *gt, void *stream,
                   dt_unet **out) {
  if (!desc || !bt || !gt || !out) return DT_E_NULL;
  if (desc->channels < 1 || desc->channels > 3 || desc->temb_dim < 2) return DT_E_SHAPE;
  for (int i = 0; i < 4; ++i)
    if (desc->dims[i] < 1) return DT_E_SHAPE;
  for (int i = 0; i < DT_GT_COUNT; ++i)
    if (!gt[i]) return DT_E_NULL;
  hipStream_t s = (hipStream_t)stream;
  dt_unet *u = new (std::nothrow) dt_unet();
  if (!u) return (int)hipErrorOutOfMemory;
  u->desc = *desc;
  u->precision = DT_PREC_AUTO;
  const int C = desc->channels, D = desc->temb_dim;
  const int *d = desc->dims;
  for (int i = 0; i < 4; ++i) u->cp[i] = round_up(d[i], kChanPad);
  const int cin[kBlocks] = {C, d[0], d[1], d[2], d[3], d[3] + d[3], d[2] + d[2], d[1] + d[1]};
  const int cout[kBlocks] = {d[0], d[1], d[2], d[3], d[3], d[2], d[1], d[0]};
  const int up_c[kBlocks] = {0, 0, 0, 0, 0, d[3], d[2], d[1]};
  Bump bump;
  size_t o_w1[kBlocks], o_w2[kBlocks], o_wr[kBlocks], o_ss[kBlocks];
  size_t o_w1b[kBlocks], o_w2b[kBlocks], o_wrb[kBlocks];
  int tb = 0;
  for (int j = 0; j < kBlocks; ++j) {
    BlockW &k = u->blk[j];
    k.cin = cin[j]; k.cout = cout[j];
    k.cout_p = round_up(cout[j], kChanPad);
    k.n_p = round_up(cout[j], kNPad);
    if (j >= 5) {
      k.split_c = up_c[j]; k.split_cp = round_up(up_c[j], kChanPad);
      k.cin_p = k.split_cp + round_up(cin[j] - up_c[j], kChanPad);
    } else {
      k.cin_p = round_up(cin[j], kChanPad);
      k.split_c = cin[j]; k.split_cp = k.cin_p;
    }
    k.has_res = cin[j] != cout[j];
    k.cin_w = round_up(k.cin_p, 16 * kChunkPad); k.cout_w = round_up(k.cout_p, 16 * kChunkPad);
    for (int t = 0; t < DT_BT_COUNT; ++t) {
      const bool optional = t == DT_BT_RES_W || t == DT_BT_RES_B;
      if (!bt[j * DT_BT_COUNT + t] && (!optional || k.has_res)) { delete u; return DT_E_NULL; }
    }
    o_w1[j] = bump.take(j == 0 ? (size_t)9 * C * k.cout_p : (size_t)9 * k.cin_p * k.n_p);
    o_w2[j] = bump.take((size_t)9 * k.cout_p * k.n_p);
    o_wr[j] = k.has_res ? bump.take(j == 0 ? (size_t)4 * k.n_p : (size_t)k.cin_p * k.n_p) : 0;
    o_ss[j] = bump.take((size_t)6 * k.n_p);
    o_w1b[j] = j == 0 ? 0 : bump.take((size_t)9 * k.cin_w * k.n_p * 3 / 2);
    o_w2b[j] = bump.take((size_t)9 * k.cout_w * k.n_p * 3 / 2);
    o_wrb[j] = (k.has_res && j > 0) ? bump.take((size_t)k.cin_w * k.n_p * 3 / 2) : 0;
    k.tb_off = tb;
    tb += k.cout_p;
  }
  u->share_enc1 = getenv("DT_NO_SHARED_ENC1") == nullptr;
  const int c0p = u->blk[0].cout_p;
  u->tb_cols = tb;
  u->tb_stride = tb + (u->share_enc1 ? 9 * c0p : 0);
  const size_t o_w2t = u->share_enc1 ? bump.take((size_t)9 * c0p * c0p) : 0;
  const int half = (D / 2 > 1 ? D / 2 : 1);
  const size_t o_wt = bump.take((size_t)tb * D), o_bt = bump.take(tb);
  const size_t o_w1g = bump.take((size_t)D * D), o_b1g = bump.take(D), o_wc0 = bump.take(D), o_bc0 = bump.take(D);
  const size_t o_wc2 = bump.take((size_t)D * D), o_bc2 = bump.take(D), o_fr = bump.take(half);
  const size_t o_fw = bump.take((size_t)C * d[0]), o_fb = bump.take(C);
  u->slab_floats = bump.off;
  hipError_t e = hipMalloc((void **)&u->slab, u->slab_floats * sizeof(float));
  if (e != hipSuccess) { delete u; return (int)e; }
  float *S = u->slab;
  int st = DT_OK;
  auto copy = [&](size_t off, const float *src, size_t n) {
    if (st == DT_OK) {
      hipError_t ee = hipMemcpyAsync(S + off, src, n * sizeof(float), hipMemcpyDeviceToDevice, s);
      if (ee != hipSuccess) st = (int)ee;
    }
  };
  for (int j = 0; j < kBlocks && st == DT_OK; ++j) {
    BlockW &k = u->blk[j];
    const float *const *t = bt + j * DT_BT_COUNT;
    k.w1 = S + o_w1[j]; k.w2 = S + o_w2[j];
    k.wr = (k.has_res && j > 0) ? S + o_wr[j] : nullptr;
    k.w3 = j == 0 ? S + o_wr[j] : nullptr;
    k.w1b = S + o_w1b[j]; k.w2b = S + o_w2b[j]; k.wrb = (k.has_res && j > 0) ? S + o_wrb[j] : nullptr;
    float *ss = S + o_ss[j];
    k.s1 = ss; k.h1 = ss + k.n_p; k.s2 = ss + 2 * k.n_p; k.h2 = ss + 3 * k.n_p; k.sr = ss + 4 * k.n_p; k.hr = ss + 5 * k.n_p;
    if (j == 0)
      st = launch_pack_first_conv(t[DT_BT_CONV1_W], k.w1, k.cout, C, k.cout_p, s);
    else
      st = launch_pack_conv(t[DT_BT_CONV1_W], k.w1, k.cout, k.cin, 3, k.cin_p, k.n_p, k.split_c, k.split_cp, s);
    if (!st) st = launch_pack_conv(t[DT_BT_CONV2_W], k.w2, k.cout, k.cout, 3, k.cout_p, k.n_p, k.cout, k.cout_p, s);
    if (!st && k.has_res && j > 0)
      st = launch_pack_conv(t[DT_BT_RES_W], k.wr, k.cout, k.cin, 1, k.cin_p, k.n_p, k.split_c, k.split_cp, s);
    if (!st && j > 0) st = launch_pack_conv_bf16x3(t[DT_BT_CONV1_W], k.w1b, k.cout, k.cin, 3, k.cin_p, k.cin_w, k.n_p, k.split_c, k.split_cp, s);
    if (!st) st = launch_pack_conv_bf16x3(t[DT_BT_CONV2_W], k.w2b, k.cout, k.cout, 3, k.cout_p, k.cout_w, k.n_p, k.cout, k.cout_p, s);
    if (!st && k.has_res && j > 0)
      st = launch_pack_conv_bf16x3(t[DT_BT_RES_W], k.wrb, k.cout, k.cin, 1, k.cin_p, k.cin_w, k.n_p, k.split_c, k.split_cp, s);
    if (!st && j == 0) st = launch_pack_res3(t[DT_BT_RES_W], t[DT_BT_RES_B], k.w3, k.cout, C, k.n_p, s);
    if (!st && j == 0 && u->share_enc1) st = launch_pack_tap_major(t[DT_BT_CONV2_W], S + o_w2t, k.cout, k.cout, k.cout_p, s);
    if (!st) st = launch_fold_bn(t[DT_BT_CONV1_B], t[DT_BT_BN1_G], t[DT_BT_BN1_B], t[DT_BT_BN1_MEAN], t[DT_BT_BN1_VAR],
                                 k.s1, k.h1, k.cout, k.n_p, s);
    if (!st) st = launch_fold_bn(t[DT_BT_CONV2_B], t[DT_BT_BN2_G], t[DT_BT_BN2_B], t[DT_BT_BN2_MEAN], t[DT_BT_BN2_VAR],
                                 k.s2, k.h2, k.cout, k.n_p, s);
    if (!st && k.has_res && j > 0)
      st = launch_fold_bn(t[DT_BT_RES_B], nullptr, nullptr, nullptr, nullptr, k.sr, k.hr, k.cout, k.n_p, s);
    if (!st) st = launch_pack_linear_rows(t[DT_BT_TIME_W], t[DT_BT_TIME_B], S + o_wt + (size_t)k.tb_off * D,
                                          S + o_bt + k.tb_off, k.cout, D, k.cout_p, s);
  }
  copy(o_w1g, gt[DT_GT_TIME1_W], (size_t)D * D); copy(o_b1g, gt[DT_GT_TIME1_B], D);
  copy(o_wc0, gt[DT_GT_COND0_W], D); copy(o_bc0, gt[DT_GT_COND0_B], D);
  copy(o_wc2, gt[DT_GT_COND2_W], (size_t)D * D); copy(o_bc2, gt[DT_GT_COND2_B], D);
  copy(o_fr, gt[DT_GT_FREQS], half);
  copy(o_fw, gt[DT_GT_FINAL_W], (size_t)C * d[0]); copy(o_fb, gt[DT_GT_FINAL_B], C);
  if (st != DT_OK) { (void)hipFree(u->slab); delete u; return st; }
  u->tw = TembWeights{S + o_fr, S + o_w1g, S + o_b1g, S + o_wc0, S + o_bc0, S + o_wc2, S + o_bc2, S + o_wt, S + o_bt,
                      D, half, u->tb_stride, tb, u->share_enc1 ? S + o_w2t : nullptr, c0p};
  u->final_w = S + o_fw; u->final_b = S + o_fb;
  st = build_fused(u, bt, s);
  if (st != DT_OK) { (void)hipFree(u->slab); if (u->fused_slab) (void)hipFree(u->fused_slab); delete u; return st; }
  *out = u;
  return DT_OK;
}

void dt_unet_destroy(dt_unet *h) {
  if (!h) return;
  drop_graphs(h);
  if (h->slab) (void)hipFree(h->slab);
  if (h->fused_slab) (void)hipFree(h->fused_slab);
  delete h;
}

int dt_unet_time_bias_stride(const dt_unet *h) { return h ? h->tb_stride : DT_E_NULL; }

int dt_unet_time_bias(const dt_unet *h, const int32_t *t, const float *cond, const uint8_t *present, int rows,
                      float *out, void *stream) {
  if (!h || !t || !out) return DT_E_NULL;
  if (rows < 0) return DT_E_ARG;
  return launch_time_bias(h->tw, t, cond, present, rows, out, (hipStream_t)stream);
}

size_t dt_unet_workspace_bytes(const dt_unet *h, int batch_total, int H, int W) {
  const FwdShape sh = FwdShape::rows_only(batch_total, H, W);
  if (!h || sh.validate() != DT_OK) return 0;
  return make_plan(h, sh).total * sizeof(float);
}

int dt_unet_forward(const dt_unet *h, const float *x, int B, int n_pass, int H, int W, const float *tb, int tb_div,
                    float *eps, void *ws, size_t ws_bytes, void *stream) {
  if (!eps) return DT_E_NULL;
  return forward_impl(h, x, B, n_pass, H, W, tb, tb_div, eps, (float *)ws, ws_bytes, (hipStream_t)stream);
}

constexpr float kSplitMargin = 1.05f;

int dt_unet_autotune(dt_unet *h, int batch_total, int H, int W, int images, int single, void *workspace, size_t ws_bytes,
                     void *stream) {
  if (!h || !workspace) return DT_E_NULL;
  TunedShape t{{batch_total, H, W, images, single}, {}};
  if (const int bad = t.shape.validate()) return bad;
  hipStream_t s = (hipStream_t)stream;
  const Plan pl = make_plan(h, t.shape);
  if (pl.total * sizeof(float) > ws_bytes) return DT_E_WORKSPACE;
  float *ws = (float *)workspace;
  ConvTimer timer;
  if (const int bad = timer.create()) return bad;
  const ResolvedForward f = resolve_forward(h, t.shape, nullptr);
  const float *tb = h->slab;
  int st = DT_OK;
  {
    const ConvParams wp = bind_conv(h, f, 1, 1, f.c[1][1], ws + pl.pool[0], ws, pl, tb, batch_total);
    for (int rep = 0; rep < 200 && st == DT_OK; ++rep) st = launch_conv(wp, s);
    if (hipStreamSynchronize(s) != hipSuccess) st = (int)hipGetLastError();
  }
  for (int j = 0; j < kBlocks && st == DT_OK; ++j) {
    const float *in = j == 0 ? ws + pl.h[0] : (j <= 4 ? ws + pl.pool[j - 1] : ws + pl.cat[j - 5]);
    float skip_ms = 0.f;
    for (int slot = 0; slot < 3 && st == DT_OK; ++slot) {
      if (!has_launch(h, j, slot)) continue;
      ConvChoice best = f.c[j][slot];
      best.fuse = 0;
      const ConvLayer L = conv_layer(h, f, j, slot);
      float best_ms = 1e30f;
      auto measure = [&](const ConvParams &q, int reps) -> float {
        float ms;
        const int lst = timer.time(q, reps, s, &ms);
        if (lst != DT_OK && lst != DT_E_SHAPE && lst != DT_E_ARG) st = lst;
        return lst == DT_OK ? ms : -1.f;
      };
      struct Cand { ConvChoice c; ConvParams q; float cost; };
      std::vector<Cand> cands;
      auto cost_of = [&](float ms, const ConvChoice &c) {
        return (ms + (c.fuse ? 0.f : (L.foldable ? skip_ms : 0.f))) * (c.splits > 1 ? kSplitMargin : 1.0f);
      };
      const bool strip_ok = L.taps == 9 && strip_reaches(L.W);
      for (const int kind : {KIND_FP32, KIND_BF16, KIND_STRIP, KIND_STRIP2, KIND_STRIPK}) {
        if (h->precision == DT_PREC_FP32 ? kind != KIND_FP32 : kind == KIND_FP32) continue;
        if (is_strip(kind) ? !strip_ok : (kind == KIND_BF16 && strip_ok)) continue;
        for (int bm = 64; bm <= 256; bm *= 2)
          for (int bn = 64; bn <= 128; bn += 64) {
            if (j == kBlocks - 1 && slot == 2 && h->head_fusion && h->desc.channels <= 3 && L.n_p <= 128 && bn != L.n_p) continue;
            const long long tiles = (long long)((L.M + bm - 1) / bm) * (L.n_p / bn);
            for (int sp = 1; sp <= (L.splittable ? 9 : 1); sp *= ((is_strip(kind) || L.taps != 9) ? 2 : 3))
              for (int fuse = 0; fuse <= ((L.foldable && sp == 1) ? 1 : 0); ++fuse) {
                if (sp > 1 && tiles * (sp / 2) >= 1024) continue;
                const ConvChoice c{bm, bn, sp, kind, fuse};
                const ConvParams q = bind_conv(h, f, j, slot, c, in, ws, pl, tb, batch_total);
                if (conv_admissible(q) != DT_OK) continue;
                const float ms = measure(q, 3);
                if (ms < 0.f) continue;
                cands.push_back(Cand{c, q, cost_of(ms, c)});
              }
          }
      }
      if (!cands.empty() && st == DT_OK) {
        std::vector<size_t> top;
        for (size_t i = 0; i < cands.size(); ++i) top.push_back(i);
        std::stable_sort(top.begin(), top.end(), [&](size_t a, size_t b) { return cands[a].cost < cands[b].cost; });
        if (top.size() > 3) top.resize(3);
        std::sort(top.begin(), top.end());
        std::vector<float> fin(top.size(), 1e30f);
        for (int round = 0; round < 2 && st == DT_OK; ++round)
          for (size_t k = 0; k < top.size() && st == DT_OK; ++k) {
            const float ms = measure(cands[top[k]].q, 10);
            if (ms >= 0.f && ms < fin[k]) fin[k] = ms;
          }
        for (size_t k = 0; k < top.size(); ++k) {
          const float cost = cost_of(fin[k], cands[top[k]].c);
          if (cost < best_ms * 1.01f) { best_ms = cost < best_ms ? cost : best_ms; best = cands[top[k]].c; }
        }
      }
      t.c[j][slot] = best;
      if (slot == 0) skip_ms = best_ms;
    }
  }
  if (st != DT_OK) return st;
  TunedShape *old = const_cast<TunedShape *>(find_tuned(h, t.shape));
  if (old) *old = t;
  else h->tuned.push_back(t);
  drop_graphs(h);
  return DT_OK;
}

int dt_unet_time_conv(const dt_unet *h, int batch_total, int H, int W, int images, int single, int block, int slot, int bm,
                      int bn, int splits, int prec, int fuse, int reps, void *workspace, size_t ws_bytes, void *stream,
                      float *ms, double *flops) {
  if (!h || !workspace || !ms || !flops) return DT_E_NULL;
  if (!slot_exists(block, slot) || reps < 1) return DT_E_ARG;
  TunedShape req{{batch_total, H, W, images, single}, {}};
  if (const int bad = req.shape.validate()) return bad;
  const Plan pl = make_plan(h, req.shape);
  if (pl.total * sizeof(float) > ws_bytes) return DT_E_WORKSPACE;
  float *ws = (float *)workspace;
  const float *in = block == 0 ? ws + pl.h[0] : (block <= 4 ? ws + pl.pool[block - 1] : ws + pl.cat[block - 5]);
  if (!has_launch(h, block, slot)) { *ms = 0.f; *flops = 0.0; return DT_OK; }
  std::fill_n(&req.c[0][0], kBlocks * 3, ConvChoice{bm, bn, splits, prec, fuse});
  const ResolvedForward f = resolve_forward(h, req.shape, &req);
  const ConvParams p = bind_conv(h, f, block, slot, f.c[block][slot], in, ws, pl, h->slab, batch_total);
  *flops = 2.0 * p.M * (double)p.cout_real * ((double)p.cin_real * p.ksize * p.ksize + (p.in2 ? p.cin2_real : 0));
  ConvTimer timer;
  if (const int bad = timer.create()) return bad;
  return timer.time(p, reps, (hipStream_t)stream, ms);
}

int dt_unet_set_precision(dt_unet *h, int precision) {
  if (!h) return DT_E_NULL;
  if (precision < DT_PREC_FP32 || precision > DT_PREC_AUTO) return DT_E_ARG;
  h->tuned.clear();
  drop_graphs(h);
  h->precision = precision;
  return DT_OK;
}

int dt_unet_set_head_fusion(dt_unet *h, int on) {
  if (!h) return DT_E_NULL;
  h->head_fusion = on != 0;
  drop_graphs(h);
  return DT_OK;
}

int dt_unet_set_fused(dt_unet *h, int on) {
  if (!h) return DT_E_NULL;
  h->fused_on = on != 0 && h->fused_ok;
  drop_graphs(h);
  return DT_OK;
}

int dt_unet_fused_active(const dt_unet *h, int H, int W) {
  if (!h) return DT_E_NULL;
  return use_fused(h, H, W) ? 1 : 0;
}

int dt_unet_conv_choice(const dt_unet *h, int batch_total, int H, int W, int images, int single, int block, int slot, int *bm,
                        int *bn, int *splits, int *prec, int *tuned) {
  if (!h || !bm || !bn || !splits || !prec || !tuned) return DT_E_NULL;
  if (!slot_exists(block, slot)) return DT_E_ARG;
  const FwdShape sh{batch_total, H, W, images, single};
  if (const int bad = sh.validate()) return bad;
  const TunedShape *t = find_tuned(h, sh);
  const ResolvedForward f = resolve_forward(h, sh, t);
  const ConvChoice &c = f.c[block][slot];
  *bm = c.bm; *bn = c.bn; *splits = c.splits; *prec = c.kind + (c.fuse ? 8 : 0); *tuned = t && has_launch(h, block, slot);
  if (slot == 0 && f.c[block][2].fuse) *bm = *bn = *splits = 0;
  return DT_OK;
}

int dt_unet_set_conv_choice(dt_unet *h, int batch_total, int H, int W, int images, int single, int block, int slot, int bm,
                            int bn, int splits, int prec, int fuse) {
  if (!h) return DT_E_NULL;
  if (!slot_exists(block, slot)) return DT_E_ARG;
  const FwdShape sh{batch_total, H, W, images, single};
  if (const int bad = sh.validate()) return bad;
  const ConvChoice c{bm, bn, splits, prec, fuse};
  if (!conv_choice_valid(c, slot, h->blk[block].n_p)) return DT_E_ARG;
  TunedShape *t = const_cast<TunedShape *>(find_tuned(h, sh));
  if (!t) {
    TunedShape fresh{sh, {}};
    memcpy(fresh.c, resolve_forward(h, sh, nullptr).c, sizeof(fresh.c));
    h->tuned.push_back(fresh);
    t = &h->tuned.back();
  }
  t->c[block][slot] = c;
  drop_graphs(h);
  return DT_OK;
}

int dt_unet_debug_activation(const dt_unet *h, int batch_total, int H, int W, int which, size_t *off, int *cp,
                             int *oh, int *ow) {
  if (!h || !off || !cp || !oh || !ow) return DT_E_NULL;
  if (which < 0 || which > kBlocks) return DT_E_ARG;
  const FwdShape sh = FwdShape::rows_only(batch_total, H, W);
  if (const int bad = sh.validate()) return bad;
  const Plan pl = make_plan(h, sh);
  if (which == kBlocks) { *off = pl.slab; *cp = 0; *oh = 0; *ow = 0; return DT_OK; }
  *off = pl.o[which]; *cp = h->blk[which].cout_p; *oh = pl.H[which]; *ow = pl.W[which];
  return DT_OK;
}

struct SampleArgs {
  int rule, B, n_pass, B_single, H, W, n_steps;
  const float *tb;
  int tb_div;
  const float *coef;
  const int32_t *has_noise;
  const float *z;
  const int32_t *z_row;
  const int64_t *z_shift;
  const float *w;
  float w_scalar;
  float *traj;
  void *ws;
  size_t ws_bytes;
  hipStream_t s;
};

static int sample_loop(const dt_unet *h, const SampleArgs &a) {
  const int B = a.B, H = a.H, W = a.W;
  const int E = h->desc.channels * H * W;
  const size_t slot = (size_t)B * E;
  const FwdShape sh{B * a.n_pass - a.B_single * (a.n_pass - 1), H, W, B, a.B_single};
  if (const int bad = sh.validate()) return bad;
  if (a.tb_div < 1 || sh.Bt % a.tb_div) return DT_E_ARG;
  const int tb_rows = sh.Bt / a.tb_div;
  const Plan pl = make_plan(h, sh);
  if (pl.total * sizeof(float) > a.ws_bytes) return DT_E_WORKSPACE;
  if (use_fused(h, H, W)) {
    for (int i0 = 0; i0 < a.n_steps; i0 += kFusedMaxSteps) {
      const int n = a.n_steps - i0 < kFusedMaxSteps ? a.n_steps - i0 : kFusedMaxSteps;
      FusedArgs fa{};
      fused_common(h, fa, B, a.n_pass, a.B_single, a.tb + (size_t)i0 * tb_rows * h->tb_stride, a.tb_div);
      fa.mode = FUSED_LOOP; fa.rule = a.rule; fa.n_steps = n;
      fa.traj = a.traj + (size_t)i0 * slot; fa.z = a.z; fa.z_row = a.z_row; fa.wg = a.w; fa.w_scalar = a.w_scalar;
      for (int i = 0; i < n; ++i) {
        fa.coef[i][0] = a.coef[4 * (i0 + i)]; fa.coef[i][1] = a.coef[4 * (i0 + i) + 1]; fa.coef[i][2] = a.coef[4 * (i0 + i) + 2];
        fa.z_shift[i] = a.z_shift ? (long long)a.z_shift[i0 + i] : 0;
        if (a.has_noise[i0 + i]) fa.noise_mask |= 1ull << i;
        if (a.has_noise[i0 + i] && !a.z) return DT_E_NULL;
      }
      const int st = launch_unet_fused(fa, a.s);
      if (st) return st;
    }
    return DT_OK;
  }
  const float *lowres = (const float *)a.ws + pl.lowres;
  for (int i = 0; i < a.n_steps; ++i) {
    const float *x = a.traj + (size_t)i * slot;
    float *xn = a.traj + (size_t)(i + 1) * slot;
    const bool dead = a.rule == DT_RULE_ENGINE && !a.has_noise[i];
    if (!dead) {
      int st = forward_impl(h, x, B, a.n_pass, H, W, a.tb + (size_t)i * tb_rows * h->tb_stride, a.tb_div, nullptr, (float *)a.ws, a.ws_bytes,
                            a.s, a.B_single);
      if (st) return st;
    }
    int st = launch_cfg_update_lowres(a.rule, x, lowres, a.n_pass == 2 ? lowres + (size_t)(B - a.B_single) * (H / 2) * (W / 2) * 4 : nullptr, a.z,
                                      a.z_row, a.z_shift ? (long long)a.z_shift[i] : 0, a.coef + 4 * i, a.has_noise[i], a.w, a.w_scalar, xn,
                                      B, h->desc.channels, H, W, a.B_single, a.s);
    if (st) return st;
  }
  return DT_OK;
}

int dt_sample_trajectory(const dt_unet *h, int rule, int B, int n_pass, int H, int W, int n_steps, const float *tb,
                         const float *coef, const int32_t *has_noise, const float *z, const int32_t *z_row,
                         const int64_t *z_shift, const float *w, float w_scalar, float *traj, void *ws, size_t ws_bytes,
                         void *stream) {
  if (!h || !tb || !coef || !has_noise || !traj || !ws) return DT_E_NULL;
  if (n_pass < 1 || n_pass > 2 || n_steps < 0 || rule < 0 || rule > DT_RULE_MANAGER) return DT_E_ARG;
  hipStream_t s = (hipStream_t)stream;
  const SampleArgs a{rule, B, n_pass, 0, H, W, n_steps, tb, B, coef, has_noise, z, z_row, z_shift, w, w_scalar, traj, ws, ws_bytes, s};
  const char *genv = getenv("DT_GRAPH");
  const bool use_graph = genv && atoi(genv) != 0;
  if (!use_graph || g_prof.on.load() || n_steps < 4) return sample_loop(h, a);
  std::vector<unsigned char> key;
  auto put = [&key](const void *p, size_t n) { const unsigned char *c = (const unsigned char *)p; key.insert(key.end(), c, c + n); };
  const int ints[7] = {a.rule, a.B, a.n_pass, a.H, a.W, a.n_steps, a.z_shift ? 1 : 0};
  const void *ptrs[7] = {a.tb, a.z, a.z_row, a.w, a.traj, a.ws, (const void *)a.s};
  put(ints, sizeof(ints)); put(ptrs, sizeof(ptrs)); put(&a.w_scalar, sizeof(a.w_scalar)); put(&a.ws_bytes, sizeof(a.ws_bytes));
  put(a.coef, sizeof(float) * 4 * n_steps); put(a.has_noise, sizeof(int32_t) * n_steps);
  if (a.z_shift) put(a.z_shift, sizeof(int64_t) * n_steps);
  const dt_unet *hm = h;
  std::lock_guard<std::mutex> lock(hm->graph_mu);
  for (const LoopGraph &g : hm->graphs)
    if (g.key == key) return (int)hipGraphLaunch(g.exec, s);
  hipError_t e = hipStreamBeginCapture(s, hipStreamCaptureModeThreadLocal);
  if (e != hipSuccess) {
    (void)hipGetLastError();
    return sample_loop(h, a);
  }
  const int st = sample_loop(h, a);
  LoopGraph g{};
  e = hipStreamEndCapture(s, &g.graph);
  if (st != DT_OK) { if (e == hipSuccess && g.graph) (void)hipGraphDestroy(g.graph); return st; }
  if (e != hipSuccess) return (int)e;
  e = hipGraphInstantiate(&g.exec, g.graph, nullptr, nullptr, 0);
  if (e != hipSuccess) { (void)hipGraphDestroy(g.graph); return (int)e; }
  g.key = std::move(key);
  if (hm->graphs.size() >= 8) { (void)hipGraphExecDestroy(hm->graphs.front().exec); (void)hipGraphDestroy(hm->graphs.front().graph); hm->graphs.erase(hm->graphs.begin()); }
  hm->graphs.push_back(std::move(g));
  if (getenv("DT_GRAPH_DEBUG")) fprintf(stderr, "[dt_hip] captured sampler loop: %d steps, batch %d -> graph #%zu\n", n_steps, B, hm->graphs.size());
  return (int)hipGraphLaunch(hm->graphs.back().exec, s);
}

int dt_sample_trajectory_mixed(const dt_unet *h, int rule, int B, int B_single, int H, int W, int n_steps, const float *tb,
                               int tb_div, const float *coef, const int32_t *has_noise, const float *z, const int32_t *z_row,
                               const int64_t *z_shift, const float *w, float *traj, void *ws, size_t ws_bytes, void *stream) {
  if (!h || !tb || !coef || !has_noise || !traj || !ws || !w) return DT_E_NULL;
  if (n_steps < 0 || rule < 0 || rule > DT_RULE_MANAGER || B < 2 || B_single < 1 || B_single >= B || tb_div < 1) return DT_E_ARG;
  if ((2 * B - B_single) % tb_div || B_single % tb_div || !h->share_enc1) return DT_E_ARG;
  return sample_loop(h, SampleArgs{rule, B, 2, B_single, H, W, n_steps, tb, tb_div, coef, has_noise, z, z_row, z_shift, w, 1.f, traj, ws, ws_bytes,
                                   (hipStream_t)stream});
}

int dt_unet_forward_mixed(const dt_unet *h, const float *x, int B, int B_single, int H, int W, const float *tb, int tb_div,
                          float *eps, void *ws, size_t ws_bytes, void *stream) {
  if (!eps || !h) return DT_E_NULL;
  if (B_single < 1 || B_single >= B || tb_div < 1 || (2 * B - B_single) % tb_div || B_single % tb_div || !h->share_enc1) return DT_E_ARG;
  return forward_impl(h, x, B, 2, H, W, tb, tb_div, eps, (float *)ws, ws_bytes, (hipStream_t)stream, B_single);
}

__global__ void profile_marker_kernel(int) {}

int dt_profile_marker(int id, void *stream) {
  profile_marker_kernel<<<1, 64, 0, (hipStream_t)stream>>>(id);
  DT_LAUNCH_CHECK();
  return DT_OK;
}

int dt_profile_begin(void) {
  std::lock_guard<std::mutex> lock(g_prof.mu);
  g_prof.rec.clear();
  g_prof.used = 0;
  g_prof.on = true;
  return DT_OK;
}

int dt_profile_end(void) {
  std::lock_guard<std::mutex> lock(g_prof.mu);
  g_prof.on = false;
  return DT_OK;
}

int dt_profile_class_count(void) { return KC_COUNT; }

int dt_profile_read(int cls, const char **name, long long *launches, double *ms, double *flops, double *bytes) {
  if (cls < 0 || cls >= KC_COUNT || !launches || !ms || !flops || !bytes) return DT_E_ARG;
  if (name) *name = class_name(cls);
  *launches = 0; *ms = 0; *flops = 0; *bytes = 0;
  std::lock_guard<std::mutex> lock(g_prof.mu);
  for (const ProfRecord &r : g_prof.rec) {
    if (r.cls != cls) continue;
    DT_HIP_TRY(hipEventSynchronize(r.b));
    float t = 0.f;
    DT_HIP_TRY(hipEventElapsedTime(&t, r.a, r.b));
    *launches += 1; *ms += t; *flops += r.flops; *bytes += r.bytes;
  }
  return DT_OK;
}

}
```

distillation_trajectories_amd/csrc/dt_update.hip:

```cpp
#include "dt_update_math.h"
#include "../../include/dt_hip_noise.h"

#pragma clang fp contract(off)

namespace dt {

struct UpdateArgs {
  const float *x, *eu, *ec, *z;
  const int32_t *z_row;
  const float *w;
  float *out;
  StepCoef k;
  float w_scalar;
  long long z_shift;
  int has_noise, B, E4;
  int lh, lw, hw;
  int b_single;
};

__device__ inline float4 eps_from_lowres(const float *lowres, int b, int e, const UpdateArgs &a) {
  const int W = 2 * a.lw, H = 2 * a.lh;
  const int idx = e * 4, c = idx / a.hw, pix = idx - c * a.hw;
  const int y = pix / W, x0 = pix - y * W;
  int y0, y1;
  float wy0, wy1;
  bilinear_src(y, a.lh, H, y0, y1, wy0, wy1);
  const float *base = lowres + (size_t)b * a.lh * a.lw * 4 + c;
  float r[4];
#pragma unroll
  for (int j = 0; j < 4; ++j) {
    int xa, xb;
    float wx0, wx1;
    bilinear_src(x0 + j, a.lw, W, xa, xb, wx0, wx1);
    const float v00 = base[((size_t)y0 * a.lw + xa) * 4], v01 = base[((size_t)y0 * a.lw + xb) * 4];
    const float v10 = base[((size_t)y1 * a.lw + xa) * 4], v11 = base[((size_t)y1 * a.lw + xb) * 4];
    r[j] = bilinear_blend(v00, v01, v10, v11, wy0, wy1, wx0, wx1);
  }
  return make_float4(r[0], r[1], r[2], r[3]);
}

template <int RULE, bool LOWRES = false>
__global__ __launch_bounds__(256) void cfg_update_kernel(const UpdateArgs a) {
  const size_t total = (size_t)a.B * a.E4;
  const float4 *x4 = reinterpret_cast<const float4 *>(a.x);
  const float4 *eu4 = reinterpret_cast<const float4 *>(a.eu);
  const float4 *ec4 = reinterpret_cast<const float4 *>(a.ec);
  const float4 *z4 = reinterpret_cast<const float4 *>(a.z);
  float4 *o4 = reinterpret_cast<float4 *>(a.out);
  for (size_t i = blockIdx.x * (size_t)blockDim.x + threadIdx.x; i < total; i += (size_t)gridDim.x * blockDim.x) {
    const int b = i / a.E4, e = i - (size_t)b * a.E4;
    const float4 xv = x4[i];
    if (RULE == DT_RULE_ENGINE && !a.has_noise) { o4[i] = xv; continue; }
    float4 ev = LOWRES ? eps_from_lowres(a.eu, b, e, a) : eu4[i];
    if (a.ec && b >= a.b_single) {
      const float4 cv = LOWRES ? eps_from_lowres(a.ec, b, e, a) : ec4[i];
      const float w = a.w ? a.w[b] : a.w_scalar;
      ev.x = ev.x + w * (cv.x - ev.x);
      ev.y = ev.y + w * (cv.y - ev.y);
      ev.z = ev.z + w * (cv.z - ev.z);
      ev.w = ev.w + w * (cv.w - ev.w);
    }
    float4 zv = make_float4(0.f, 0.f, 0.f, 0.f);
    const bool noise = a.has_noise != 0;
    if (noise) {
      const long long zr = (a.z_row ? (long long)a.z_row[b] : (long long)b) + a.z_shift;
      zv = z4[(size_t)zr * a.E4 + e];
    }
    float4 o;
    if (RULE != DT_RULE_PSAMPLE && !noise) {
      o.x = step1<RULE>(xv.x, ev.x, 0.f, a.k, false); o.y = step1<RULE>(xv.y, ev.y, 0.f, a.k, false);
      o.z = step1<RULE>(xv.z, ev.z, 0.f, a.k, false); o.w = step1<RULE>(xv.w, ev.w, 0.f, a.k, false);
    } else {
      o.x = step1<RULE>(xv.x, ev.x, zv.x, a.k, noise); o.y = step1<RULE>(xv.y, ev.y, zv.y, a.k, noise);
      o.z = step1<RULE>(xv.z, ev.z, zv.z, a.k, noise); o.w = step1<RULE>(xv.w, ev.w, zv.w, a.k, noise);
    }
    o4[i] = o;
  }
}

extern "C" int dt_cfg_update(int rule, const float *x, const float *eu, const float *ec, const float *z, const int32_t *z_row,
                             const float coef[4], int has_noise, const float *w, float w_scalar, float *out, int B, int E,
                             void *stream) {
  hipStream_t s = (hipStream_t)stream;
  if (!x || !eu || !out || !coef) return DT_E_NULL;
  if (has_noise && !z) return DT_E_NULL;
  if (B <= 0 || E <= 0 || E % 4) return DT_E_SHAPE;
  UpdateArgs a{x, eu, ec, z, z_row, w, out, {coef[0], coef[1], coef[2]}, w_scalar, 0, has_noise, B, E / 4, 0, 0, 0, 0};
  const size_t total = (size_t)B * (E / 4);
  const int blocks = (int)((total + 255) / 256 < 2048 ? (total + 255) / 256 : 2048);
  ProfileScope prof(KC_UPDATE, 0.0, 4.0 * B * E * (2.0 + (has_noise ? 1.0 : 0.0) + (ec ? 2.0 : 1.0)), s);
  switch (rule) {
    case DT_RULE_ENGINE: cfg_update_kernel<DT_RULE_ENGINE><<<blocks, 256, 0, s>>>(a); break;
    case DT_RULE_PSAMPLE: cfg_update_kernel<DT_RULE_PSAMPLE><<<blocks, 256, 0, s>>>(a); break;
    case DT_RULE_MANAGER: cfg_update_kernel<DT_RULE_MANAGER><<<blocks, 256, 0, s>>>(a); break;
    default: return DT_E_ARG;
  }
  DT_LAUNCH_CHECK();
  return DT_OK;
}

int launch_cfg_update_lowres(int rule, const float *x, const float *lowres_u, const float *lowres_c, const float *z,
                             const int32_t *z_row, long long z_shift, const float coef[4], int has_noise, const float *w,
                             float w_scalar, float *out, int B, int C, int H, int W, int b_single, hipStream_t s) {
  if (!x || !lowres_u || !out || !coef) return DT_E_NULL;
  if (has_noise && !z) return DT_E_NULL;
  const int E = C * H * W;
  if (B <= 0 || E <= 0 || W % 4 || H % 2 || W % 2) return DT_E_SHAPE;
  if (b_single < 0 || b_single > B) return DT_E_ARG;
  UpdateArgs a{x, lowres_u, lowres_c, z, z_row, w, out, {coef[0], coef[1], coef[2]}, w_scalar, z_shift, has_noise, B, E / 4,
               H / 2, W / 2, H * W, b_single};
  const size_t total = (size_t)B * (E / 4);
  const int blocks = (int)((total + 255) / 256 < 2048 ? (total + 255) / 256 : 2048);
  ProfileScope prof(KC_UPDATE, 0.0, 4.0 * B * E * (2.0 + (has_noise ? 1.0 : 0.0)) + 4.0 * B * H * W * (lowres_c ? 2.0 : 1.0), s);
  switch (rule) {
    case DT_RULE_ENGINE: cfg_update_kernel<DT_RULE_ENGINE, true><<<blocks, 256, 0, s>>>(a); break;
    case DT_RULE_PSAMPLE: cfg_update_kernel<DT_RULE_PSAMPLE, true><<<blocks, 256, 0, s>>>(a); break;
    case DT_RULE_MANAGER: cfg_update_kernel<DT_RULE_MANAGER, true><<<blocks, 256, 0, s>>>(a); break;
    default: return DT_E_ARG;
  }
  DT_LAUNCH_CHECK();
  return DT_OK;
}

__global__ __launch_bounds__(256) void q_sample_kernel(const float4 *x0, const float4 *z, const float2 *coef, size_t be4,
                                                       size_t total, float4 *out) {
  for (size_t i = blockIdx.x * (size_t)blockDim.x + threadIdx.x; i < total; i += (size_t)gridDim.x * blockDim.x) {
    const size_t g = i / be4;
    const float2 c = coef[g];
    const float4 xv = x0[i - g * be4], zv = z[i];
    float4 o;
    o.x = c.x * xv.x + c.y * zv.x;
    o.y = c.x * xv.y + c.y * zv.y;
    o.z = c.x * xv.z + c.y * zv.z;
    o.w = c.x * xv.w + c.y * zv.w;
    out[i] = o;
  }
}

extern "C" int dt_q_sample(const float *x0, const float *z, const float *coef, int n_groups, int B, int E, float *out, void *stream) {
  hipStream_t s = (hipStream_t)stream;
  if (!x0 || !z || !coef || !out) return DT_E_NULL;
  if (n_groups <= 0 || B <= 0 || E <= 0 || E % 4) return DT_E_SHAPE;
  if (((uintptr_t)x0 | (uintptr_t)z | (uintptr_t)out) & 15 || (uintptr_t)coef & 7) return DT_E_ARG;
  const size_t be4 = (size_t)B * (E / 4), total = (size_t)n_groups * be4;
  const int blocks = (int)((total + 255) / 256 < 2048 ? (total + 255) / 256 : 2048);
  ProfileScope prof(KC_UPDATE, 3.0 * 4 * total, 4.0 * 4 * be4 * (2.0 * n_groups + 1.0), s);
  q_sample_kernel<<<blocks, 256, 0, s>>>(reinterpret_cast<const float4 *>(x0), reinterpret_cast<const float4 *>(z),
                                         reinterpret_cast<const float2 *>(coef), be4, total, reinterpret_cast<float4 *>(out));
  DT_LAUNCH_CHECK();
  return DT_OK;
}

}
```

distillation_trajectories_amd/csrc/dt_update_math.h:

```cpp
#pragma once
#include "dt_internal.h"

namespace dt {

struct StepCoef { float c0, c1, c2; };

template <int RULE>
__device__ inline float step1(float x, float eps, float z, const StepCoef &a, bool noise) {
#pragma clang fp contract(off)
  if (RULE == DT_RULE_ENGINE) {
    const float v = a.c0 * x - a.c1 * eps;
    return v + a.c2 * z;
  } else if (RULE == DT_RULE_PSAMPLE) {
    const float v = a.c0 * (x - a.c1 * eps);
    return v + (noise ? z * a.c2 : 0.f * a.c2);
  } else {
    const float v = (x - a.c0 * eps) / a.c1;
    return v + a.c2 * z;
  }
}

__device__ inline float step1_rt(int rule, float x, float eps, float z, const StepCoef &a, bool noise) {
  if (rule == DT_RULE_ENGINE) return step1<DT_RULE_ENGINE>(x, eps, z, a, noise);
  if (rule == DT_RULE_PSAMPLE) return step1<DT_RULE_PSAMPLE>(x, eps, z, a, noise);
  return step1<DT_RULE_MANAGER>(x, eps, z, a, noise);
}

__device__ inline float cfg_mix(float eu, float ec, float w) {
#pragma clang fp contract(off)
  return eu + w * (ec - eu);
}

__device__ inline float eps_at(const float *lowres, int lh, int lw, int c, int y, int x) {
  int y0, y1, xa, xb;
  float wy0, wy1, wx0, wx1;
  bilinear_src(y, lh, 2 * lh, y0, y1, wy0, wy1);
  bilinear_src(x, lw, 2 * lw, xa, xb, wx0, wx1);
  const float *base = lowres + c;
  const float v00 = base[(y0 * lw + xa) * 4], v01 = base[(y0 * lw + xb) * 4];
  const float v10 = base[(y1 * lw + xa) * 4], v11 = base[(y1 * lw + xb) * 4];
  return bilinear_blend(v00, v01, v10, v11, wy0, wy1, wx0, wx1);
}

}
```

Before: 357,600.

## Fuse bilinear upsample+concat into conv epilogues and update step into first conv

Adds an upsample-and-concat pass to the conv GEMM epilogue and to the split-K epilogue, so decoder blocks write the upsampled tensor and skip channels directly and no separate upcat kernel is launched. The trajectory loop also defers the per-step sampler update and merges it into the next step's first convolution, which computes x_next while loading pixels and writes it out. Both changes cut kernel launches and global round-trips per timestep. The cost is more complex epilogues: a serial per-thread upsample loop in the split-K path, an extra LDS sync, and a modified blend order that must still match the reference.

Result: no change. 355,700 (-0.5%).

```diff
diff --git a/distillation_trajectories_amd/csrc/dt_conv.hip b/distillation_trajectories_amd/csrc/dt_conv.hip
--- a/distillation_trajectories_amd/csrc/dt_conv.hip
+++ b/distillation_trajectories_amd/csrc/dt_conv.hip
@@ -192,6 +192,7 @@
   return f->reaches(p.W) ? DT_OK : DT_E_SHAPE;
 }
 
+enum { FIN_PLAIN, FIN_POOL, FIN_UP };
 template <int S>
 __device__ inline float4 splitk_finish(const ConvParams &p, unsigned m, int n, size_t slab_stride) {
   const size_t o = (size_t)m * p.cout_p + n;
@@ -225,11 +226,43 @@
   return v;
 }
 
-template <int S, bool POOL>
+template <int S, int FIN>
 __global__ __launch_bounds__(256) void splitk_epilogue_kernel(const ConvParams p) {
   const unsigned c4 = (unsigned)p.cout_p >> 2;
   const size_t slab_stride = (size_t)p.M * p.cout_p;
-  if (!POOL) {
+  if (FIN == FIN_UP) {
+    const unsigned HW = (unsigned)(p.H * p.W), Wo = 2u * p.W, Ho = 2u * p.H;
+    const unsigned total = ((unsigned)p.M / HW) * c4;
+    for (unsigned i = blockIdx.x * blockDim.x + threadIdx.x; i < total; i += gridDim.x * blockDim.x) {
+      const unsigned b = i / c4;
+      const int n = (int)(i - b * c4) * 4;
+      float4 v[4];
+#pragma unroll
+      for (unsigned k = 0; k < 4; ++k) v[k] = k < HW ? splitk_finish<S>(p, b * HW + k, n, slab_stride) : make_float4(0.f, 0.f, 0.f, 0.f);
+      const float scale_y = bilinear_scale(p.H, (int)Ho), scale_x = bilinear_scale(p.W, (int)Wo);
+      auto at = [&](int k) {
+        const float4 a = v[0], b1 = v[1], c = v[2], d = v[3];
+        return make_float4(k == 0 ? a.x : (k == 1 ? b1.x : (k == 2 ? c.x : d.x)), k == 0 ? a.y : (k == 1 ? b1.y : (k == 2 ? c.y : d.y)),
+                           k == 0 ? a.z : (k == 1 ? b1.z : (k == 2 ? c.z : d.z)), k == 0 ? a.w : (k == 1 ? b1.w : (k == 2 ? c.w : d.w)));
+      };
+      for (unsigned Y = 0; Y < Ho; ++Y) {
+        int y0, y1;
+        float wy0, wy1;
+        bilinear_src_scaled((int)Y, p.H, scale_y, y0, y1, wy0, wy1);
+        for (unsigned X = 0; X < Wo; ++X) {
+          int x0, x1;
+          float wx0, wx1;
+          bilinear_src_scaled((int)X, p.W, scale_x, x0, x1, wx0, wx1);
+          const size_t opix = ((size_t)b * Ho + Y) * Wo + X;
+          float *o = p.up_out + opix * p.up_stride;
+          *reinterpret_cast<float4 *>(o + n) = upcat_blend(at(y0 * p.W + x0), at(y0 * p.W + x1), at(y1 * p.W + x0), at(y1 * p.W + x1), wy0, wy1, wx0, wx1);
+          if (p.up_skip)
+            for (int q = n; q < p.up_skip_c; q += p.cout_p)
+              *reinterpret_cast<float4 *>(o + p.cout_p + q) = *reinterpret_cast<const float4 *>(p.up_skip + opix * p.up_skip_c + q);
+        }
+      }
+    }
+  } else if (FIN == FIN_PLAIN) {
     const unsigned total = (unsigned)p.M * c4;
     const bool pow2 = (c4 & (c4 - 1)) == 0;
     const int sh4 = 31 - __builtin_clz(c4);
@@ -256,11 +289,11 @@
   }
 }
 
-template <bool POOL>
+template <int POOL>
 static int launch_splitk_epilogue_t(const ConvParams &p, hipStream_t s) {
-  const size_t total = (size_t)(POOL ? p.M / 4 : p.M) * (p.cout_p / 4);
+  const size_t total = (size_t)(POOL == FIN_POOL ? p.M / 4 : (POOL == FIN_UP ? p.M / (p.H * p.W) : p.M)) * (p.cout_p / 4);
   const int blocks = (int)((total + 255) / 256 < 4096 ? (total + 255) / 256 : 4096);
-  ProfileScope prof(KC_SPLITK_EPILOGUE, 0.0, 4.0 * p.M * p.cout_p * (p.splits + 1.0 + (POOL ? 0.25 : 0.0)), s);
+  ProfileScope prof(KC_SPLITK_EPILOGUE, 0.0, 4.0 * p.M * p.cout_p * (p.splits + 1.0 + (POOL == FIN_POOL ? 0.25 : (POOL == FIN_UP ? 4.0 : 0.0))), s);
   switch (p.splits) {
     case 2: splitk_epilogue_kernel<2, POOL><<<blocks, 256, 0, s>>>(p); break;
     case 3: splitk_epilogue_kernel<3, POOL><<<blocks, 256, 0, s>>>(p); break;
@@ -274,7 +307,8 @@
 }
 
 int launch_splitk_epilogue(const ConvParams &p, hipStream_t s) {
-  return p.pool_out ? launch_splitk_epilogue_t<true>(p, s) : launch_splitk_epilogue_t<false>(p, s);
+  if (p.up_out) return p.H * p.W <= 4 && !p.pool_out ? launch_splitk_epilogue_t<FIN_UP>(p, s) : DT_E_ARG;
+  return p.pool_out ? launch_splitk_epilogue_t<FIN_POOL>(p, s) : launch_splitk_epilogue_t<FIN_PLAIN>(p, s);
 }
 
 __global__ void pack_conv_kernel(const float *__restrict__ w, float *__restrict__ wp, int cout, int cin, int ksize,
diff --git a/distillation_trajectories_amd/csrc/dt_conv_epilogue.h b/distillation_trajectories_amd/csrc/dt_conv_epilogue.h
--- a/distillation_trajectories_amd/csrc/dt_conv_epilogue.h
+++ b/distillation_trajectories_amd/csrc/dt_conv_epilogue.h
@@ -111,6 +111,33 @@
       *reinterpret_cast<f32x4 *>(pool_out + pass * out_pitch + (((size_t)bimg * (p.H >> 1) + (y >> 1)) * Wo + (x >> 1)) * p.cout_p + qn) = mx;
     }
   };
+  auto up_pass = [&](int mi) __attribute__((always_inline)) {
+    __syncthreads();
+    const int Wo = 2 * p.W, px_sh = hw_sh + 2;
+    const float scale_y = bilinear_scale(p.H, 2 * p.H), scale_x = bilinear_scale(p.W, Wo);
+    for (int q0 = tid; q0 < WM * 128 * C4; q0 += 256) {
+      const int qc = q0 % C4, pp = q0 / C4;
+      const int g = pp >> 7, j = pp & 127;
+      const int pic = j >> px_sh, r = j & ((1 << px_sh) - 1);
+      const int Y = r >> (w_sh + 1), X = r & (Wo - 1);
+      const int mpic = m0 + g * (MI * 32) + mi * 32 + pic * HW;
+      const int qn = n0 + qc * 4;
+      if (mpic >= p.M || qn >= p.cout_p) continue;
+      int y0, y1, x0, x1;
+      float wy0, wy1, wx0, wx1;
+      bilinear_src_scaled(Y, p.H, scale_y, y0, y1, wy0, wy1);
+      bilinear_src_scaled(X, p.W, scale_x, x0, x1, wx0, wx1);
+      const float *s0 = stage + (g * 32 + pic * HW) * P + qc * 4;
+      const float4 v00 = *reinterpret_cast<const float4 *>(s0 + (y0 * p.W + x0) * P), v01 = *reinterpret_cast<const float4 *>(s0 + (y0 * p.W + x1) * P);
+      const float4 v10 = *reinterpret_cast<const float4 *>(s0 + (y1 * p.W + x0) * P), v11 = *reinterpret_cast<const float4 *>(s0 + (y1 * p.W + x1) * P);
+      const size_t opix = ((size_t)(mpic >> hw_sh) << px_sh) + r;
+      float *o = p.up_out + opix * p.up_stride;
+      *reinterpret_cast<float4 *>(o + qn) = upcat_blend(v00, v01, v10, v11, wy0, wy1, wx0, wx1);
+      if (p.up_skip)
+        for (int q = qn; q < p.up_skip_c; q += p.cout_p)
+          *reinterpret_cast<float4 *>(o + p.cout_p + q) = *reinterpret_cast<const float4 *>(p.up_skip + opix * p.up_skip_c + q);
+    }
+  };
   f32x4 w3r[4];
 #pragma unroll
   for (int e = 0; e < 4; ++e) w3r[e] = p.x3 ? *reinterpret_cast<const f32x4 *>(p.w3 + 4 * (nn + e)) : f32x4{0.f, 0.f, 0.f, 0.f};
@@ -292,6 +319,11 @@
       for (int k = 0; k < U; ++k) *reinterpret_cast<f32x4 *>(stage + (row0 + k * (256 / C4)) * P + c4 * 4) = v[k];
       pool_pass(mi, p.pool_out, stage, 1, 0, 0);
     }
+    if (p.up_out) {
+#pragma unroll
+      for (int k = 0; k < U; ++k) *reinterpret_cast<f32x4 *>(stage + (row0 + k * (256 / C4)) * P + c4 * 4) = v[k];
+      up_pass(mi);
+    }
   }
 }
 
diff --git a/distillation_trajectories_amd/csrc/dt_internal.h b/distillation_trajectories_amd/csrc/dt_internal.h
--- a/distillation_trajectories_amd/csrc/dt_internal.h
+++ b/distillation_trajectories_amd/csrc/dt_internal.h
@@ -21,7 +21,7 @@
 
 enum KernelClass {
   KC_SPLITK_EPILOGUE = KC_CONV_COUNT, KC_FIRST_CONV, KC_POOL, KC_UPCAT, KC_HEAD, KC_HEAD_UP, KC_TIME_BIAS, KC_UPDATE, KC_METRICS,
-  KC_WASSERSTEIN, KC_RESAMPLE, KC_FUSED, KC_PAIR_METRICS,
+  KC_WASSERSTEIN, KC_RESAMPLE, KC_FUSED, KC_PAIR_METRICS, KC_UPDATE_FIRST_CONV,
   KC_COUNT
 };
 struct ProfileScope {
@@ -32,18 +32,37 @@
   void *end_event;
 };
 
-__device__ inline void bilinear_src(int dst, int in, int out, int &i0, int &i1, float &l0, float &l1) {
+__device__ inline float bilinear_scale(int in, int out) { return out > 1 ? (float)(in - 1) / (float)(out - 1) : 0.f; }
+__device__ inline void bilinear_src_scaled(int dst, int in, float scale, int &i0, int &i1, float &l0, float &l1) {
 #pragma clang fp contract(off)
-  const float scale = out > 1 ? (float)(in - 1) / (float)(out - 1) : 0.f;
   const float src = scale * (float)dst;
   i0 = (int)src;
   i1 = i0 + (i0 < in - 1 ? 1 : 0);
   l1 = src - (float)i0;
   l0 = 1.f - l1;
 }
+__device__ inline void bilinear_src(int dst, int in, int out, int &i0, int &i1, float &l0, float &l1) {
+  bilinear_src_scaled(dst, in, bilinear_scale(in, out), i0, i1, l0, l1);
+}
 __device__ inline float bilinear_blend(float v00, float v01, float v10, float v11, float wy0, float wy1, float wx0, float wx1) {
   const float top = fmaf(wx1, v01, wx0 * v00), bot = fmaf(wx1, v11, wx0 * v10);
   return fmaf(wy1, bot, wy0 * top);
+}
+
+template <bool ODD>
+__device__ inline float upcat_blend1(float v00, float v01, float v10, float v11, float wy0, float wy1, float wx0, float wx1) {
+#pragma clang fp contract(off)
+  if (ODD) {
+    const float top = fmaf(wx1, v01, wx0 * v00), bot = fmaf(wx1, v11, wx0 * v10);
+    return fmaf(wy0, top, wy1 * bot);
+  }
+  const float top = fmaf(wx0, v00, wx1 * v01), bot = fmaf(wx0, v10, wx1 * v11);
+  return fmaf(wy1, bot, wy0 * top);
+}
+__device__ inline float4 upcat_blend(const float4 &v00, const float4 &v01, const float4 &v10, const float4 &v11, float wy0, float wy1,
+                                     float wx0, float wx1) {
+  return make_float4(upcat_blend1<false>(v00.x, v01.x, v10.x, v11.x, wy0, wy1, wx0, wx1), upcat_blend1<true>(v00.y, v01.y, v10.y, v11.y, wy0, wy1, wx0, wx1),
+                     upcat_blend1<false>(v00.z, v01.z, v10.z, v11.z, wy0, wy1, wx0, wx1), upcat_blend1<true>(v00.w, v01.w, v10.w, v11.w, wy0, wy1, wx0, wx1));
 }
 
 constexpr int kChanPad = 16;
@@ -93,6 +112,9 @@
   int dup_skip;
   int skip_out;
   int dup_stage2;
+  float *up_out;
+  const float *up_skip;
+  int up_stride, up_skip_c;
   int ccw, ccw2;
 };
 
@@ -132,6 +154,10 @@
 
 int launch_first_conv(const float *x, const float *wf, const float *scale, const float *shift, const float *tb, int tb_stride,
                       int tb_div, float *out, int B, int n_pass, int C, int H, int W, int cout, int cout_p, hipStream_t s);
+int launch_update_first_conv(int rule, const float *x, const float *lowres_u, const float *lowres_c, const float *z,
+                             const int32_t *z_row, long long z_shift, const float coef[4], int has_noise, const float *w,
+                             float w_scalar, float *x_next, int b_single, const float *wf, const float *scale, const float *shift,
+                             float *out, int B, int C, int H, int W, int cout, int cout_p, hipStream_t s);
 int launch_pack_first_conv(const float *w_oihw, float *wf, int cout, int C, int cout_p, hipStream_t s);
 int launch_pack_tap_major(const float *w_oihw, float *w2t, int cout, int cin, int cp, hipStream_t s);
 int launch_maxpool(const float *in, float *out, int Bt, int H, int W, int cp, hipStream_t s);
diff --git a/distillation_trajectories_amd/csrc/dt_layers.hip b/distillation_trajectories_amd/csrc/dt_layers.hip
--- a/distillation_trajectories_amd/csrc/dt_layers.hip
+++ b/distillation_trajectories_amd/csrc/dt_layers.hip
@@ -1,33 +1,61 @@
 #include "dt_conv_epilogue.h"
+#include "dt_update_math.h"
 
 namespace dt {
 
-template <int C, int PX>
-__global__ __launch_bounds__(256) void first_conv_kernel(const float *__restrict__ x, const float *__restrict__ wf,
-                                                         const float *__restrict__ scale, const float *__restrict__ shift,
-                                                         const float *__restrict__ tb, int tb_stride, int tb_div,
-                                                         float *__restrict__ out, int B, int n_pass, int H, int W, int cp,
-                                                         int parts) {
-  extern __shared__ float img[];
-  const int tid = threadIdx.x, b = blockIdx.x / parts, part = blockIdx.x - b * parts;
+struct FirstConvArgs {
+  const float *wf, *scale, *shift, *tb;
+  int tb_stride, tb_div;
+  float *out;
+  int B, n_pass, H, W, cp, parts;
+};
+
+template <int C, int PX, typename Pixel, typename Keep>
+__device__ inline void first_conv_body(const FirstConvArgs &a, float *img, int b, int part, Pixel pixel, Keep keep) {
+  const float *__restrict__ wf = a.wf, *__restrict__ tb = a.tb;
+  float *__restrict__ out = a.out;
+  const int tb_stride = a.tb_stride, tb_div = a.tb_div, B = a.B, n_pass = a.n_pass, H = a.H, W = a.W, cp = a.cp, parts = a.parts;
+  const int tid = threadIdx.x;
   const int Wp = W + 2, plane = (H + 2) * Wp, HW = H * W;
   const int QN = cp >> 2, PPI = 256 / QN;
   const int q = tid % QN, pl = tid / QN;
+  const int GW = W / PX, G = H * GW;
+  const int per = (G + parts - 1) / parts;
+  const int lo = part * per, hi = (part + 1) * per < G ? (part + 1) * per : G;
   f32x4 w[9 * C];
 #pragma unroll
   for (int k = 0; k < 9 * C; ++k) w[k] = *reinterpret_cast<const f32x4 *>(wf + (size_t)k * cp + q * 4);
-  const f32x4 sc = *reinterpret_cast<const f32x4 *>(scale + q * 4), sh = *reinterpret_cast<const f32x4 *>(shift + q * 4);
-  for (int i = tid; i < C * plane; i += 256) {
-    const int c = i / plane, r = i - c * plane;
-    const int y = r / Wp - 1, xx = r - (y + 1) * Wp - 1;
-    img[i] = (y >= 0 && y < H && xx >= 0 && xx < W) ? x[((size_t)(b * C + c) * H + y) * W + xx] : 0.f;
+  const f32x4 sc = *reinterpret_cast<const f32x4 *>(a.scale + q * 4), sh = *reinterpret_cast<const f32x4 *>(a.shift + q * 4);
+  if (lo < hi) {
+    const int r_lo = lo / GW, rows = (hi - 1) / GW + 3 - r_lo;
+    const int n = C * rows * Wp;
+    constexpr int UF = 4;
+    for (int i0 = tid; i0 < n; i0 += 256 * UF) {
+      float v[UF];
+      int cc[UF], yy[UF], xx[UF], at[UF];
+      bool in[UF];
+#pragma unroll
+      for (int u = 0; u < UF; ++u) {
+        const int i = i0 + u * 256, c = i / (rows * Wp), r = i - c * (rows * Wp);
+        const int ry = r / Wp, rx = r - ry * Wp;
+        cc[u] = c; yy[u] = r_lo + ry - 1; xx[u] = rx - 1;
+        at[u] = c * plane + (r_lo + ry) * Wp + rx;
+        in[u] = i < n && yy[u] >= 0 && yy[u] < H && xx[u] >= 0 && xx[u] < W;
+        v[u] = in[u] ? pixel(cc[u], yy[u], xx[u]) : 0.f;
+      }
+#pragma unroll
+      for (int u = 0; u < UF; ++u) {
+        if (i0 + u * 256 < n) img[at[u]] = v[u];
+        if (in[u]) {
+          const int g = yy[u] * GW + xx[u] / PX;
+          keep(cc[u], yy[u], xx[u], v[u], g >= lo && g < hi);
+        }
+      }
+    }
   }
   __syncthreads();
   if (pl >= PPI) return;
-  const int GW = W / PX, G = H * GW;
-  const int per = (G + parts - 1) / parts;
-  const int hi = (part + 1) * per < G ? (part + 1) * per : G;
-  for (int g = part * per + pl; g < hi; g += PPI) {
+  for (int g = lo + pl; g < hi; g += PPI) {
     const int y = g / GW, x0 = (g - y * GW) * PX;
     f32x4 acc[PX];
 #pragma unroll
@@ -61,26 +89,73 @@
   }
 }
 
-template <int PX>
-static void first_conv_dispatch(int C, int grid, size_t lds, hipStream_t s, const float *x, const float *wf, const float *scale,
-                                const float *shift, const float *tb, int tb_stride, int tb_div, float *out, int B, int n_pass,
-                                int H, int W, int cout_p, int parts) {
-  if (C == 1) first_conv_kernel<1, PX><<<grid, 256, lds, s>>>(x, wf, scale, shift, tb, tb_stride, tb_div, out, B, n_pass, H, W, cout_p, parts);
-  else if (C == 2) first_conv_kernel<2, PX><<<grid, 256, lds, s>>>(x, wf, scale, shift, tb, tb_stride, tb_div, out, B, n_pass, H, W, cout_p, parts);
-  else first_conv_kernel<3, PX><<<grid, 256, lds, s>>>(x, wf, scale, shift, tb, tb_stride, tb_div, out, B, n_pass, H, W, cout_p, parts);
-}
-
-int launch_first_conv(const float *x, const float *wf, const float *scale, const float *shift, const float *tb, int tb_stride,
-                      int tb_div, float *out, int B, int n_pass, int C, int H, int W, int cout, int cout_p, hipStream_t s) {
+template <int C, int PX>
+__global__ __launch_bounds__(256) void first_conv_kernel(const float *__restrict__ x, const FirstConvArgs a) {
+  extern __shared__ float img[];
+  const int b = blockIdx.x / a.parts, part = blockIdx.x - b * a.parts;
+  first_conv_body<C, PX>(a, img, b, part, [&](int c, int y, int xx) { return x[((size_t)(b * C + c) * a.H + y) * a.W + xx]; },
+                         [](int, int, int, float, bool) {});
+}
+
+template <int C, int PX, int RULE>
+__global__ __launch_bounds__(256) void update_first_conv_kernel(const UpdateArgs u, const FirstConvArgs a) {
+  extern __shared__ float img[];
+  const int b = blockIdx.x / a.parts, part = blockIdx.x - b * a.parts;
+  first_conv_body<C, PX>(a, img, b, part,
+                         [&](int c, int y, int xx) { return update_at<RULE>(u, b, c, y, xx, u.x[((size_t)(b * C + c) * a.H + y) * a.W + xx]); },
+                         [&](int c, int y, int xx, float v, bool mine) { if (mine) u.out[((size_t)(b * C + c) * a.H + y) * a.W + xx] = v; });
+}
+
+template <int C, int PX>
+static void first_conv_dispatch(int rule, int grid, size_t lds, hipStream_t s, const float *x, const UpdateArgs &u, const FirstConvArgs &a) {
+  if (rule < 0) first_conv_kernel<C, PX><<<grid, 256, lds, s>>>(x, a);
+  else if (rule == DT_RULE_ENGINE) update_first_conv_kernel<C, PX, DT_RULE_ENGINE><<<grid, 256, lds, s>>>(u, a);
+  else if (rule == DT_RULE_PSAMPLE) update_first_conv_kernel<C, PX, DT_RULE_PSAMPLE><<<grid, 256, lds, s>>>(u, a);
+  else update_first_conv_kernel<C, PX, DT_RULE_MANAGER><<<grid, 256, lds, s>>>(u, a);
+}
+
+static int first_conv_launch(int rule, const float *x, const UpdateArgs &u, const float *wf, const float *scale, const float *shift,
+                             const float *tb, int tb_stride, int tb_div, float *out, int B, int n_pass, int C, int H, int W, int cout_p,
+                             hipStream_t s) {
   if (C < 1 || C > 3 || cout_p % 4 || cout_p > 1024) return DT_E_SHAPE;
   const size_t lds = (size_t)C * (H + 2) * (W + 2) * sizeof(float);
   if (lds > 64 * 1024) return DT_E_SHAPE;
   const int parts = B >= 1024 ? 1 : (B >= 256 ? 4 : 8);
+  const FirstConvArgs a{wf, scale, shift, tb, tb_stride, tb_div, out, B, n_pass, H, W, cout_p, parts};
+  const int grid = B * parts;
+  if (W % 4 == 0) {
+    if (C == 1) first_conv_dispatch<1, 4>(rule, grid, lds, s, x, u, a);
+    else if (C == 2) first_conv_dispatch<2, 4>(rule, grid, lds, s, x, u, a);
+    else first_conv_dispatch<3, 4>(rule, grid, lds, s, x, u, a);
+  } else {
+    if (C == 1) first_conv_dispatch<1, 1>(rule, grid, lds, s, x, u, a);
+    else if (C == 2) first_conv_dispatch<2, 1>(rule, grid, lds, s, x, u, a);
+    else first_conv_dispatch<3, 1>(rule, grid, lds, s, x, u, a);
+  }
+  DT_LAUNCH_CHECK();
+  return DT_OK;
+}
+
+int launch_first_conv(const float *x, const float *wf, const float *scale, const float *shift, const float *tb, int tb_stride,
+                      int tb_div, float *out, int B, int n_pass, int C, int H, int W, int cout, int cout_p, hipStream_t s) {
   ProfileScope prof(KC_FIRST_CONV, 2.0 * n_pass * B * H * W * (double)cout * 9 * C, 4.0 * B * H * W * (C + (double)n_pass * cout_p), s);
-  if (W % 4 == 0) first_conv_dispatch<4>(C, B * parts, lds, s, x, wf, scale, shift, tb, tb_stride, tb_div, out, B, n_pass, H, W, cout_p, parts);
-  else first_conv_dispatch<1>(C, B * parts, lds, s, x, wf, scale, shift, tb, tb_stride, tb_div, out, B, n_pass, H, W, cout_p, parts);
-  DT_LAUNCH_CHECK();
-  return DT_OK;
+  return first_conv_launch(-1, x, UpdateArgs{}, wf, scale, shift, tb, tb_stride, tb_div, out, B, n_pass, C, H, W, cout_p, s);
+}
+
+int launch_update_first_conv(int rule, const float *x, const float *lowres_u, const float *lowres_c, const float *z,
+                             const int32_t *z_row, long long z_shift, const float coef[4], int has_noise, const float *w,
+                             float w_scalar, float *x_next, int b_single, const float *wf, const float *scale, const float *shift,
+                             float *out, int B, int C, int H, int W, int cout, int cout_p, hipStream_t s) {
+  if (!x || !lowres_u || !x_next || !coef || !wf || !scale || !shift || !out) return DT_E_NULL;
+  if (has_noise && !z) return DT_E_NULL;
+  if (rule < DT_RULE_ENGINE || rule > DT_RULE_MANAGER || b_single < 0 || b_single > B) return DT_E_ARG;
+  if (B <= 0 || H % 2 || W % 2) return DT_E_SHAPE;
+  const int E = C * H * W;
+  const UpdateArgs u{x, lowres_u, lowres_c, z, z_row, w, x_next, {coef[0], coef[1], coef[2]}, w_scalar, z_shift, has_noise, B, E / 4,
+                     H / 2, W / 2, H * W, b_single};
+  ProfileScope prof(KC_UPDATE_FIRST_CONV, 2.0 * B * H * W * (double)cout * 9 * C,
+                    4.0 * B * E * (2.0 + (has_noise ? 1.0 : 0.0)) + 4.0 * B * H * W * ((lowres_c ? 2.0 : 1.0) + cout_p), s);
+  return first_conv_launch(rule, x, u, wf, scale, shift, nullptr, 0, 1, out, B, 1, C, H, W, cout_p, s);
 }
 
 __global__ void pack_first_conv_kernel(const float *__restrict__ w, float *__restrict__ wf, int cout, int C, int cp) {
@@ -147,10 +222,7 @@
       const float4 *base = lo + (size_t)b * h * w * c1q + c;
       const float4 v00 = base[(y0 * w + x0) * c1q], v01 = base[(y0 * w + x1) * c1q];
       const float4 v10 = base[(y1 * w + x0) * c1q], v11 = base[(y1 * w + x1) * c1q];
-      o.x = wy0 * (wx0 * v00.x + wx1 * v01.x) + wy1 * (wx0 * v10.x + wx1 * v11.x);
-      o.y = wy0 * (wx0 * v00.y + wx1 * v01.y) + wy1 * (wx0 * v10.y + wx1 * v11.y);
-      o.z = wy0 * (wx0 * v00.z + wx1 * v01.z) + wy1 * (wx0 * v10.z + wx1 * v11.z);
-      o.w = wy0 * (wx0 * v00.w + wx1 * v01.w) + wy1 * (wx0 * v10.w + wx1 * v11.w);
+      o = upcat_blend(v00, v01, v10, v11, wy0, wy1, wx0, wx1);
     }
     out[(size_t)pixel * cq + c] = o;
   }
diff --git a/distillation_trajectories_amd/csrc/dt_unet.hip b/distillation_trajectories_amd/csrc/dt_unet.hip
--- a/distillation_trajectories_amd/csrc/dt_unet.hip
+++ b/distillation_trajectories_amd/csrc/dt_unet.hip
@@ -32,7 +32,7 @@
 const char *kClassName[KC_COUNT - KC_CONV_COUNT] = {
     "splitk_epilogue_kernel", "first_conv_kernel", "maxpool_kernel", "upcat_kernel", "head_kernel", "head_upsample_kernel",
     "time_bias_kernel", "cfg_update_kernel", "traj_metrics_kernel", "wasserstein_kernel", "resampled_distance_kernel",
-    "unet_fused_kernel", "pair_metrics_kernel"};
+    "unet_fused_kernel", "pair_metrics_kernel", "update_first_conv_kernel"};
 const char *class_name(int cls) {
   switch (cls) {
 #define DT_GEMM(c, kind, bm, bn, kc, wk) case c: return "conv_gemm_kernel<" #bm "," #bn ">";
@@ -109,6 +109,7 @@
   int precision;
   bool head_fusion = true;
   bool share_enc1 = true;
+  bool fused_upsample = true, fused_update = true;
   int tb_cols = 0;
   dt_unet_desc desc;
   BlockW blk[kBlocks];
@@ -190,6 +191,7 @@
   ConvChoice c[kBlocks][3];
   bool pool_fused[kBlocks];
   bool concat_in_place[kBlocks];
+  bool up_fused[kBlocks];
   bool head_fused;
 };
 
@@ -201,6 +203,13 @@
   const int M = (j == 0 && f.shared_enc1 ? f.shape.imgs : f.shape.Bt) * h * w;
   const int taps = slot == 0 || (h == 1 && w == 1) ? 1 : 9;
   return ConvLayer{M, w, k.n_p, slot == 2 ? k.cout_p : k.cin_p, taps, j > 0 && M <= kSplitMaxRows, slot == 2 && j > 0 && k.has_res};
+}
+
+bool up_fusable(const dt_unet *u, const FwdShape &sh, int j, const ConvChoice &c) {
+  if (!u->fused_upsample || j < 4 || j > 6) return false;
+  const int h = sh.H / kDiv[j], w = sh.W / kDiv[j], hw = h * w;
+  if (c.splits > 1) return hw <= 4;
+  return c.kind != KIND_FP32 && hw <= 32 && (w & (w - 1)) == 0 && (hw & (hw - 1)) == 0;
 }
 
 ResolvedForward resolve_forward(const dt_unet *u, const FwdShape &sh, const TunedShape *tuned) {
@@ -215,6 +224,7 @@
     const int h = sh.H / kDiv[j], w = sh.W / kDiv[j];
     f.pool_fused[j] = j <= 3 && h % 2 == 0 && w % 2 == 0 && (c2.splits > 1 || (w <= 16 && (w & (w - 1)) == 0));
     f.concat_in_place[j] = j >= 5 && u->blk[j].has_res && is_strip(f.c[j][1].kind) && is_strip(c2.kind) && c2.fuse;
+    f.up_fused[j] = j >= 5 && up_fusable(u, sh, j - 1, f.c[j - 1][2]);
   }
   const ConvChoice &last = f.c[kBlocks - 1][2];
   f.head_fused = u->head_fusion && last.splits == 1 && u->blk[kBlocks - 1].n_p == last.bn && u->desc.channels <= 3;
@@ -252,6 +262,11 @@
     } else {
       p.add = k.has_res ? ws + pl.r[j] : in;
     }
+    if (up_fusable(u, f.shape, j, c)) {
+      const int skip = 7 - j;
+      p.up_out = ws + pl.cat[j - 4]; p.up_stride = u->blk[j + 1].cin_p;
+      if (!f.concat_in_place[j + 1]) { p.up_skip = ws + pl.o[skip]; p.up_skip_c = u->blk[skip].cout_p; }
+    }
     if (j == kBlocks - 1 && f.head_fused) {
       p.head_w = u->final_w; p.head_b = u->final_b; p.head_out = ws + pl.lowres;
       p.head_c = u->desc.channels; p.head_cin = u->desc.dims[0];
@@ -270,8 +285,8 @@
 }
 
 int run_block(const dt_unet *u, const ResolvedForward &f, int j, const float *in, float *ws, const Plan &pl, const float *tb,
-              int tb_div, hipStream_t s) {
-  if (j == 0) {
+              int tb_div, hipStream_t s, bool first_done) {
+  if (j == 0 && !first_done) {
     const BlockW &k = u->blk[0];
     if (!f.shared_enc1 && f.shape.single) return DT_E_ARG;
     const int st = launch_first_conv(in, k.w1, k.s1, k.h1, f.shared_enc1 ? nullptr : tb + k.tb_off, u->tb_stride, tb_div, ws + pl.h[0],
@@ -295,7 +310,7 @@
 }
 
 int forward_impl(const dt_unet *u, const float *x, int B, int n_pass, int H, int W, const float *tb, int tb_div,
-                 float *eps, float *ws, size_t ws_bytes, hipStream_t s, int B_single = 0) {
+                 float *eps, float *ws, size_t ws_bytes, hipStream_t s, int B_single = 0, bool first_done = false) {
   if (!u || !x || !tb || !ws) return DT_E_NULL;
   if (n_pass < 1 || tb_div < 1) return DT_E_SHAPE;
   const int Bt = B * n_pass - B_single * (n_pass - 1);
@@ -322,12 +337,13 @@
       cur = ws + pl.pool[j - 1];
     } else if (j >= 5) {
       const int skip = 8 - j;
+      if (!f.up_fused[j])
       st = launch_upcat(ws + pl.o[j - 1], f.concat_in_place[j] ? nullptr : ws + pl.o[skip], ws + pl.cat[j - 5],
                         Bt, pl.H[j - 1], pl.W[j - 1], u->blk[j - 1].cout_p, u->blk[skip].cout_p, s);
       if (st) return st;
       cur = ws + pl.cat[j - 5];
     }
-    st = run_block(u, f, j, cur, ws, pl, tb, tb_div, s);
+    st = run_block(u, f, j, cur, ws, pl, tb, tb_div, s, first_done);
     if (st) return st;
   }
   if (!f.head_fused) {
@@ -514,6 +530,8 @@
     tb += k.cout_p;
   }
   u->share_enc1 = getenv("DT_NO_SHARED_ENC1") == nullptr;
+  u->fused_upsample = getenv("DT_NO_FUSED_UPSAMPLE") == nullptr;
+  u->fused_update = getenv("DT_NO_FUSED_UPDATE") == nullptr;
   const int c0p = u->blk[0].cout_p;
   u->tb_cols = tb;
   u->tb_stride = tb + (u->share_enc1 ? 9 * c0p : 0);
@@ -840,18 +858,30 @@
     return DT_OK;
   }
   const float *lowres = (const float *)a.ws + pl.lowres;
+  const float *lowres_c = a.n_pass == 2 ? lowres + (size_t)(B - a.B_single) * (H / 2) * (W / 2) * 4 : nullptr;
+  auto dead = [&](int i) { return a.rule == DT_RULE_ENGINE && !a.has_noise[i]; };
+  const ResolvedForward f = resolve_forward(h, sh, find_tuned(h, sh));
+  const bool fuse_update = h->fused_update && f.shared_enc1 && f.head_fused;
+  const BlockW &k0 = h->blk[0];
+  bool deferred = false;
   for (int i = 0; i < a.n_steps; ++i) {
     const float *x = a.traj + (size_t)i * slot;
     float *xn = a.traj + (size_t)(i + 1) * slot;
-    const bool dead = a.rule == DT_RULE_ENGINE && !a.has_noise[i];
-    if (!dead) {
+    if (!dead(i)) {
+      if (deferred) {
+        const int st = launch_update_first_conv(a.rule, x - slot, lowres, lowres_c, a.z, a.z_row, a.z_shift ? (long long)a.z_shift[i - 1] : 0,
+                                                a.coef + 4 * (i - 1), a.has_noise[i - 1], a.w, a.w_scalar, a.traj + (size_t)i * slot, a.B_single,
+                                                k0.w1, k0.s1, k0.h1, (float *)a.ws + pl.h[0], B, h->desc.channels, H, W, k0.cout, k0.cout_p, a.s);
+        if (st) return st;
+      }
       int st = forward_impl(h, x, B, a.n_pass, H, W, a.tb + (size_t)i * tb_rows * h->tb_stride, a.tb_div, nullptr, (float *)a.ws, a.ws_bytes,
-                            a.s, a.B_single);
+                            a.s, a.B_single, deferred);
       if (st) return st;
     }
-    int st = launch_cfg_update_lowres(a.rule, x, lowres, a.n_pass == 2 ? lowres + (size_t)(B - a.B_single) * (H / 2) * (W / 2) * 4 : nullptr, a.z,
-                                      a.z_row, a.z_shift ? (long long)a.z_shift[i] : 0, a.coef + 4 * i, a.has_noise[i], a.w, a.w_scalar, xn,
-                                      B, h->desc.channels, H, W, a.B_single, a.s);
+    deferred = fuse_update && !dead(i) && i + 1 < a.n_steps && !dead(i + 1);
+    if (deferred) continue;
+    int st = launch_cfg_update_lowres(a.rule, x, lowres, lowres_c, a.z, a.z_row, a.z_shift ? (long long)a.z_shift[i] : 0, a.coef + 4 * i,
+                                      a.has_noise[i], a.w, a.w_scalar, xn, B, h->desc.channels, H, W, a.B_single, a.s);
     if (st) return st;
   }
   return DT_OK;
diff --git a/distillation_trajectories_amd/csrc/dt_update.hip b/distillation_trajectories_amd/csrc/dt_update.hip
--- a/distillation_trajectories_amd/csrc/dt_update.hip
+++ b/distillation_trajectories_amd/csrc/dt_update.hip
@@ -4,19 +4,6 @@
 #pragma clang fp contract(off)
 
 namespace dt {
-
-struct UpdateArgs {
-  const float *x, *eu, *ec, *z;
-  const int32_t *z_row;
-  const float *w;
-  float *out;
-  StepCoef k;
-  float w_scalar;
-  long long z_shift;
-  int has_noise, B, E4;
-  int lh, lw, hw;
-  int b_single;
-};
 
 __device__ inline float4 eps_from_lowres(const float *lowres, int b, int e, const UpdateArgs &a) {
   const int W = 2 * a.lw, H = 2 * a.lh;
diff --git a/distillation_trajectories_amd/csrc/dt_update_math.h b/distillation_trajectories_amd/csrc/dt_update_math.h
--- a/distillation_trajectories_amd/csrc/dt_update_math.h
+++ b/distillation_trajectories_amd/csrc/dt_update_math.h
@@ -42,4 +42,32 @@
   return bilinear_blend(v00, v01, v10, v11, wy0, wy1, wx0, wx1);
 }
 
+struct UpdateArgs {
+  const float *x, *eu, *ec, *z;
+  const int32_t *z_row;
+  const float *w;
+  float *out;
+  StepCoef k;
+  float w_scalar;
+  long long z_shift;
+  int has_noise, B, E4;
+  int lh, lw, hw;
+  int b_single;
+};
+
+template <int RULE>
+__device__ inline float update_at(const UpdateArgs &a, int b, int c, int y, int x, float xv) {
+  if (RULE == DT_RULE_ENGINE && !a.has_noise) return xv;
+  const size_t img = (size_t)b * a.lh * a.lw * 4;
+  float ev = eps_at(a.eu + img, a.lh, a.lw, c, y, x);
+  if (a.ec && b >= a.b_single) ev = cfg_mix(ev, eps_at(a.ec + img, a.lh, a.lw, c, y, x), a.w ? a.w[b] : a.w_scalar);
+  const bool noise = a.has_noise != 0;
+  float zv = 0.f;
+  if (noise) {
+    const long long zr = (a.z_row ? (long long)a.z_row[b] : (long long)b) + a.z_shift;
+    zv = a.z[(size_t)zr * a.E4 * 4 + (size_t)c * a.hw + y * 2 * a.lw + x];
+  }
+  return step1<RULE>(xv, ev, zv, a.k, noise);
 }
+
+}
```
